# Mictronics/pluto-gps-sim

Hardware: AMD Instinct MI355X
Metric: IQ samples/sec (whole node) at 16 channels; bit-exact int16 IQ vs CPU ref (higher is better)
Workload: dtype f64 NCOs (exact), i32 accumulate of packed int16 I/Q

## Files before the change

### pluto-gps-sim_amd/csrc/gpsbb.hip

```cpp
#include <hip/hip_runtime.h>

#include <algorithm>
#include <atomic>
#include <cctype>
#include <cmath>
#include <cstdio>
#include <cstdlib>
#include <cstring>
#include <new>
#include <condition_variable>
#include <functional>
#include <mutex>
#include <thread>
#include <chrono>
#include <vector>

#include "gpsbb.h"
#include "gpsbb_kernels.hip.h"
#include "gpsbb_noise.hip.h"
#include "gpsbb_interf.hip.h"
#include "gpsbb_level.hip.h"
#include "gpsbb_events.hip.h"
#include "gpsbb_dense.hip.h"
#include "gpsbb_despread.hip.h"
#include "gpsbb_despread_lags.hip.h"
#include "gpsbb_acq.hip.h"
#include "gpsbb_track.hip.h"
#include "gpsbb_fir.hip.h"
#include "gpsbb_psd.hip.h"
#include "gpsbb_exc.hip.h"
#include "gpsbb_blank.hip.h"
#include "gpsbb_walk.hip.h"
#include "gpsbb_laps.hip.h"
#include "gpsbb_nco.h"
#include "gpsbb_testhooks.h"
#ifdef GPSBB_EXPERIMENTS
#include "gpsbb_modelerr.hip.h"
#endif

using namespace gpsbb_impl;

#ifdef GPSBB_EXPERIMENTS
#define GPSBB_KNOB_LONG(name, dflt) ([](long d) -> long { static const char *const e = getenv(name); return e ? atol(e) : d; }((long)(dflt)))
#define GPSBB_KNOB_SET(name) ([]() -> bool { static const bool v = getenv(name) != nullptr; return v; }())
#else
#define GPSBB_KNOB_LONG(name, dflt) ((long)(dflt))
#define GPSBB_KNOB_SET(name) (false)
#endif


namespace {

constexpr uint64_t kSinCosFnv1a = 0x1c99a5cf84551314ull;

bool make_sincos(int32_t sin512[512], int32_t cos512[512])
{
    const double two_pi = 6.283185307179586476925286766559;
    for (int i = 0; i < 512; i++) {
        const double a = two_pi * (double)i / 512.0;
        sin512[i] = (int32_t)(511.0 * std::sin(a) + 1.0);
        cos512[i] = (int32_t)(511.0 * std::cos(a) + 1.0);
    }
    uint64_t h = 0xcbf29ce484222325ull;
    auto eat = [&h](const int32_t *t) {
        for (int i = 0; i < 512; i++)
            for (int k = 0; k < 4; k++) {
                h ^= (uint8_t)((uint32_t)t[i] >> (8 * k));
                h *= 0x100000001b3ull;
            }
    };
    eat(sin512);
    eat(cos512);
    return h == kSinCosFnv1a;
}

const uint8_t kG2Taps[32][2] = {
    {2, 6}, {3, 7}, {4, 8}, {5, 9}, {1, 9}, {2, 10}, {1, 8}, {2, 9}, {3, 10}, {2, 3}, {3, 4},
    {5, 6}, {6, 7}, {7, 8}, {8, 9}, {9, 10}, {1, 4}, {2, 5}, {3, 6}, {4, 7}, {5, 8}, {6, 9},
    {1, 3}, {4, 6}, {5, 7}, {6, 8}, {7, 9}, {8, 10}, {1, 6}, {2, 7}, {3, 8}, {4, 9}};

void make_ca(int prn, uint8_t ca[GPSBB_CA_LEN])
{
    uint32_t g1 = 0x3ff, g2 = 0x3ff;
// ... 388 lines not shown
};

struct Event {
    hipEvent_t e = nullptr;
    hipError_t make(unsigned flags)
    {
        if (e)
            return hipSuccess;
        const hipError_t rc = hipEventCreateWithFlags(&e, flags);
        if (rc != hipSuccess)
            e = nullptr;
        else
            live_add(g_live_events, 1);
        return rc;
    }
    void release()
    {
        if (e) {
            (void)hipEventDestroy(e);
            live_add(g_live_events, -1);
        }
        e = nullptr;
    }
    operator hipEvent_t() const { return e; }
};

template <class... B>
static void release_all(B &...b)
{
    (b.release(), ...);
}

template <class F>
struct AtExit { F f; ~AtExit() { f(); } };
template <class F> AtExit(F) -> AtExit<F>;

struct KernelTimer {
    Event ev[2];
    hipError_t start(hipStream_t stream)
    {
#ifdef GPSBB_EXPERIMENTS
        for (Event &e : ev) {
            const hipError_t rc = e.make(hipEventDefault);
            if (rc != hipSuccess)
                return rc;
        }
        return hipEventRecord(ev[0], stream);
#else
        return hipSuccess;
#endif
    }
    hipError_t stop(hipStream_t stream)
    {
#ifdef GPSBB_EXPERIMENTS
        return hipEventRecord(ev[1], stream);
#else
        return hipSuccess;
#endif
    }
    float ms() const
    {
        float t = -1.0f;
        return ev[0] && ev[1] && hipEventElapsedTime(&t, ev[0], ev[1]) == hipSuccess ? t : -1.0f;
    }
    void release() { release_all(ev[0], ev[1]); }
};

struct gpsbb {
    int device = 0;
    hipStream_t s_seed = nullptr;
    hipStream_t s_more[SEED_STREAMS_MAX - 1] = {};
    unsigned batches_created = 0;
    hipStream_t s_compute = nullptr;
    hipStream_t s_compute2 = nullptr;
    unsigned compute_turn = 0;
    hipStream_t s_copy = nullptr;
    hipStream_t s_digest = nullptr;
    std::vector<uint32_t> h_ca;
    unsigned long long host_dwrd_oob = 0, host_itable_512 = 0;
    WorkPool *pool = nullptr;
    DevBuf<int32_t> d_tabs;
    DevBuf<uint32_t> d_ca;
    DevBuf<uint32_t> d_status;
    DevBuf<unsigned long long> d_hz;
    DevBuf<unsigned long long> d_clip;
    DevBuf<int2> d_noise_tab;
    DevBuf<unsigned long long> d_nclip;
    int last_hip = 0;
    gpsbb_batch *scratch = nullptr;
    PinnedBuf<unsigned char> h_bounce;
    PinnedBuf<unsigned char> h_fill;
    struct HostReg { char *host; char *dev; size_t bytes; };
    std::vector<HostReg> host_regs;
    struct ChainOnly *chain_only = nullptr;
    int sm_count = 0;
    int opt_seed_where = 0;
    int opt_synth_kernel = 0;
    int opt_skip_seed = 0;
    int opt_chain_where = 0;
    int last_kernel = 0;
    int last_variant = 0;
    int last_chain_dev = 0;
    int last_prepass = 0;
    DevBuf<unsigned char> d_pack;
    DevBuf<LevelOut> d_level;
    DevBuf<unsigned long long> d_digest;
    DevBuf<unsigned long long> d_acq_chips, d_acq_rows;
    DevBuf<unsigned long long> d_acq_grid;
    DevBuf<unsigned long long> d_trk;
    DevBuf<unsigned long long> d_fir;
    DevBuf<unsigned long long> d_psd_tab;
    DevBuf<unsigned long long> d_psd;
    DevBuf<unsigned long long> d_exc;
    DevBuf<unsigned long long> d_blank;
    KernelTimer acq_tm, trk_tm, fir_tm, psd_tm, exc_tm, blank_tm;
};

template <class F>
static void for_each_stream(const gpsbb *h, F f)
{
    for (hipStream_t st : {h->s_seed, h->s_compute, h->s_compute2, h->s_copy, h->s_digest})
        if (st)
            f(st);
    for (hipStream_t st : h->s_more)
        if (st)
            f(st);
}

static hipError_t drain_streams(const gpsbb *h)
{
    hipError_t first = hipSuccess;
    for_each_stream(h, [&](hipStream_t st) {
        const hipError_t e = hipStreamSynchronize(st);
        if (first == hipSuccess)
            first = e;
    });
    return first;
}

struct LapScratch {
    DevBuf<LapBC> bc;
    DevBuf<uint32_t> lane0, cnt, chunk_bad;
    DevBuf<LapRec> rec;
    DevBuf<LapAgg> agg;
    DevBuf<double> chunk_m;
    int reserve(size_t nbc, size_t nch, size_t nblocks, size_t chunks, bool room)
    {
        const size_t more = room ? chunks / 4 : 0;
        int e = bc.reserve(2 * nbc);
        e = e ? e : lane0.reserve(2 * nch * (nblocks + 1));
        e = e ? e : cnt.reserve(4 * GPSBB_MAX_CHAN);
        e = e ? e : rec.reserve(chunks * LAP_WG, room ? chunks * LAP_WG / 4 : 0);
        e = e ? e : agg.reserve(chunks, more);
        e = e ? e : chunk_m.reserve(chunks, more);
        return e ? e : chunk_bad.reserve(chunks, more);
    }
    void release() { release_all(bc, lane0, cnt, chunk_bad, rec, agg, chunk_m); }
    void dev(LapDev &L) const
    {
        L.bc = bc.p;
        L.lane0 = lane0.p;
        L.nlaps = cnt.p;
        L.nbad = cnt.p + 2 * GPSBB_MAX_CHAN;
        L.rec = rec.p;
        L.agg = agg.p;
        L.chunk_m = chunk_m.p;
// ... 242 lines not shown
        *out = (uint64_t)h->last_variant;
        return GPSBB_OK;
    case GPSBB_INFO_EXACT_RUNS:
    case GPSBB_INFO_CHAIN_FALLBACKS:
    case GPSBB_INFO_CHAIN_TIES:
    case GPSBB_INFO_CHAIN_REPAIRS:
    case GPSBB_INFO_TILES_RENDERED: {
        HIPCHK(h, hipSetDevice(h->device));
        unsigned long long v = 0;
        HIPCHK(h, hipMemcpy(&v, h->d_hz.p + (what == GPSBB_INFO_EXACT_RUNS ? 2 : (what == GPSBB_INFO_CHAIN_FALLBACKS ? 4 : (what == GPSBB_INFO_CHAIN_TIES ? 5 : (what == GPSBB_INFO_TILES_RENDERED ? 7 : 6)))), 8,
                            hipMemcpyDeviceToHost));
        *out = v;
        return GPSBB_OK;
    }
    case GPSBB_INFO_SC8_CLIPPED: {
        HIPCHK(h, hipSetDevice(h->device));
        unsigned long long v = 0;
        HIPCHK(h, hipMemcpy(&v, h->d_clip.p, 8, hipMemcpyDeviceToHost));
        *out = v;
        return GPSBB_OK;
    }
    case GPSBB_INFO_NOISE_CLIPPED: {
        unsigned long long v = 0;
        if (h->d_nclip.p) {
            HIPCHK(h, hipSetDevice(h->device));
            HIPCHK(h, hipMemcpy(&v, h->d_nclip.p, 8, hipMemcpyDeviceToHost));
        }
        *out = v;
        return GPSBB_OK;
    }
    case GPSBB_INFO_CHAIN_ON_DEVICE:
        *out = (uint64_t)h->last_chain_dev;
        return GPSBB_OK;
    case GPSBB_INFO_PREPASS:
        *out = (uint64_t)h->last_prepass;
        return GPSBB_OK;
    case GPSBB_INFO_STREAMS: {
        uint64_t n = 1;
        for_each_stream(h, [&](hipStream_t) { n++; });
        *out = n;
        return GPSBB_OK;
    }
    case GPSBB_INFO_HW_QUEUES: {
        const char *e = getenv("GPU_MAX_HW_QUEUES");
        const long v = e ? atol(e) : 4;
        *out = (uint64_t)(v > 0 ? v : 4);
        return GPSBB_OK;
    }
    default:
        return GPSBB_E_BADARG;
    }
}

extern "C" int gpsbb_codegen(int prn, uint8_t ca[GPSBB_CA_LEN])
{
    if (!ca || prn < 1 || prn > 32)
        return GPSBB_E_BADARG;
    make_ca(prn, ca);
    return GPSBB_OK;
}

extern "C" int gpsbb_sincos_tables(int32_t sin512[512], int32_t cos512[512])
{
    if (!sin512 || !cos512)
        return GPSBB_E_BADARG;
    return make_sincos(sin512, cos512) ? GPSBB_OK : GPSBB_E_INTERNAL;
}

static void chain_only_free(gpsbb *h);

extern "C" void gpsbb_destroy(gpsbb_t *h)
{
    if (!h)
        return;
    (void)hipSetDevice(h->device);
    if (h->scratch)
        gpsbb_batch_destroy(h->scratch);
    release_all(h->h_fill, h->h_bounce);
    for (const gpsbb::HostReg &r : h->host_regs)
        (void)hipHostUnregister(r.host);
    h->host_regs.clear();
    chain_only_free(h);
    (void)drain_streams(h);
    release_all(h->d_tabs, h->d_ca, h->d_status, h->d_hz, h->d_clip, h->d_noise_tab, h->d_nclip);
    release_all(h->d_pack, h->d_level, h->d_digest, h->d_acq_chips, h->d_acq_rows, h->d_acq_grid, h->d_trk, h->d_fir, h->d_psd_tab, h->d_psd, h->d_exc, h->d_blank);
    release_all(h->acq_tm, h->trk_tm, h->fir_tm, h->psd_tm, h->exc_tm, h->blank_tm);
    delete h->pool;
    h->pool = nullptr;
    for_each_stream(h, [](hipStream_t st) { (void)hipStreamDestroy(st); });
    delete h;
}

static hipError_t create_seed_stream(hipStream_t *st);

#ifdef GPSBB_EXPERIMENTS
__global__ void k_park(unsigned long long ticks)
{
    const unsigned long long t0 = wall_clock64();
    while (wall_clock64() - t0 < ticks)
        __builtin_amdgcn_s_sleep(64);
}
#endif

static hipError_t zero_now(gpsbb *h, void *ptr, size_t bytes)
{
#ifdef GPSBB_EXPERIMENTS
    {
        const long park = GPSBB_KNOB_LONG("GPSBB_X_PARK_NULL_MS", 0);
        if (park > 0)
            hipLaunchKernelGGL(k_park, dim3(1), dim3(1), 0, nullptr, (unsigned long long)park * 100000ull);
        if (GPSBB_KNOB_SET("GPSBB_X_NULL_MEMSET"))
            return hipMemsetAsync(ptr, 0, bytes, nullptr);
    }
#endif
    const hipError_t e = hipMemsetAsync(ptr, 0, bytes, h->s_seed);
    return e != hipSuccess ? e : hipStreamSynchronize(h->s_seed);
}

struct SynthKernel {
    void (*fn)(BatchDev, int16_t *);
    int lds;
};
static const SynthKernel &synth_kernel(int variant, bool digest, int g);

extern "C" int gpsbb_create(gpsbb_t **out, int device)
{
    if (!out)
        return GPSBB_E_BADARG;
    *out = nullptr;
    int ndev = 0;
    if (hipGetDeviceCount(&ndev) != hipSuccess || ndev <= 0 || device < 0 || device >= ndev)
        return GPSBB_E_NODEVICE;

    int32_t tabs[1024];
    if (!make_sincos(tabs + 512, tabs))
        return GPSBB_E_INTERNAL;
    std::vector<uint32_t> ca(33 * 32, 0u);
    for (int prn = 1; prn <= 32; prn++) {
        uint8_t chips[GPSBB_CA_LEN];
        make_ca(prn, chips);
        for (int i = 0; i < GPSBB_CA_LEN; i++)
            if (chips[i])
                ca[prn * 32 + (i >> 5)] |= 1u << (i & 31);
    }

    gpsbb *h = new (std::nothrow) gpsbb;
    if (!h)
        return GPSBB_E_NOMEM;
    h->device = device;
    auto fail = [&](hipError_t e) {
        h->last_hip = (int)e;
        gpsbb_destroy(h);
        return e == hipErrorOutOfMemory ? GPSBB_E_NOMEM : GPSBB_E_HIP;
    };
    hipError_t e;
    if ((e = hipSetDevice(device)) != hipSuccess) return fail(e);
    hipDeviceProp_t prop;
    if ((e = hipGetDeviceProperties(&prop, device)) != hipSuccess) return fail(e);
    h->sm_count = prop.multiProcessorCount;
    if ((e = create_seed_stream(&h->s_seed)) != hipSuccess) return fail(e);
    {
        const long sp = GPSBB_KNOB_LONG("GPSBB_SYNTH_STREAM_PRIO", 0);
        if (sp != 0) {
            if ((e = hipStreamCreateWithPriority(&h->s_compute, hipStreamNonBlocking, (int)sp)) != hipSuccess) return fail(e);
        } else {
            if ((e = hipStreamCreateWithFlags(&h->s_compute, hipStreamNonBlocking)) != hipSuccess) return fail(e);
        }
    }
    if ((e = create_seed_stream(&h->s_more[0])) != hipSuccess) return fail(e);
    if ((e = (hipError_t)h->d_tabs.reserve(sizeof tabs / sizeof tabs[0])) != hipSuccess) return fail(e);
    if ((e = (hipError_t)h->d_ca.reserve(ca.size())) != hipSuccess) return fail(e);
    if ((e = (hipError_t)h->d_status.reserve(1)) != hipSuccess) return fail(e);
    if ((e = (hipError_t)h->d_hz.reserve(8)) != hipSuccess) return fail(e);
    if ((e = (hipError_t)h->d_clip.reserve(1)) != hipSuccess) return fail(e);
    if ((e = hipMemcpy(h->d_tabs.p, tabs, sizeof tabs, hipMemcpyHostToDevice)) != hipSuccess) return fail(e);
    if ((e = hipMemcpy(h->d_ca.p, ca.data(), ca.size() * 4, hipMemcpyHostToDevice)) != hipSuccess) return fail(e);
    if ((e = hipStreamSynchronize(nullptr)) != hipSuccess) return fail(e);
    h->h_ca = ca;
    if ((e = zero_now(h, h->d_status.p, 4)) != hipSuccess) return fail(e);
    if ((e = zero_now(h, h->d_hz.p, h->d_hz.cap * sizeof *h->d_hz.p)) != hipSuccess) return fail(e);
    if ((e = zero_now(h, h->d_clip.p, 8)) != hipSuccess) return fail(e);
    for (int v = GPSBB_VARIANT_SYNTH; v <= GPSBB_VARIANT_EV_FIXED; v++)
        for (int dg = 0; dg < 2; dg++)
            for (int g = 0; g <= EV_STATE_LOG2_MAX; g++) {
                const SynthKernel &k = synth_kernel(v, dg != 0, g);
                if (k.fn && (e = hipFuncSetAttribute(reinterpret_cast<const void *>(k.fn), hipFuncAttributeMaxDynamicSharedMemorySize,
                                                     k.lds)) != hipSuccess) return fail(e);
            }
    *out = h;
    return GPSBB_OK;
}

typedef void (*LapKernelFn)(BatchDev, LapDev);
static LapKernelFn lap_pass2_kernel(int kind, bool wide, int g)
{
#define GPSBB_P2(W) {{k_lap_pass2<NCO_CODE, W, 0>, k_lap_pass2<NCO_CODE, W, 1>, k_lap_pass2<NCO_CODE, W, 2>}, \
                     {k_lap_pass2<NCO_CARR, W, 0>, k_lap_pass2<NCO_CARR, W, 1>, k_lap_pass2<NCO_CARR, W, 2>}, \
                     {k_lap_pass2_2<W, 0>, k_lap_pass2_2<W, 1>, k_lap_pass2_2<W, 2>}}
    static const LapKernelFn k[2][3][EV_STATE_LOG2_MAX + 1] = {GPSBB_P2(false), GPSBB_P2(true)};
#undef GPSBB_P2
    static_assert(NCO_CODE == 0 && NCO_CARR == 1, "lap_pass2_kernel's table");
    return k[wide ? 1 : 0][kind < 0 ? 2 : kind][g];
}

static const SynthKernel &synth_kernel(int variant, bool digest, int g)
{
#define GPSBB_SK(v, k) {k, synth_lds(v)}
#define GPSBB_SK1(v, k) {GPSBB_SK(v, k), {}, {}}
    static const SynthKernel k[GPSBB_VARIANT_EV_FIXED + 1][2][EV_STATE_LOG2_MAX + 1] = {
        {},
        {GPSBB_SK1(GPSBB_VARIANT_SYNTH, k_synth), {}},
        {{GPSBB_SK(GPSBB_VARIANT_EV, k_synth_ev<0>), GPSBB_SK(GPSBB_VARIANT_EV, k_synth_ev<1>), GPSBB_SK(GPSBB_VARIANT_EV, k_synth_ev<2>)},
         {GPSBB_SK(GPSBB_VARIANT_EV, k_synth_ev_digest<0>), GPSBB_SK(GPSBB_VARIANT_EV, k_synth_ev_digest<1>),
          GPSBB_SK(GPSBB_VARIANT_EV, k_synth_ev_digest<2>)}},
        {GPSBB_SK1(GPSBB_VARIANT_EV_DENSE, k_synth_ev_dense), {}},
        {GPSBB_SK1(GPSBB_VARIANT_PD_WIDE, k_synth_pd<true>), GPSBB_SK1(GPSBB_VARIANT_PD_WIDE, (k_synth_pd<true, true>))},
        {GPSBB_SK1(GPSBB_VARIANT_PD_NARROW, k_synth_pd<false>), GPSBB_SK1(GPSBB_VARIANT_PD_NARROW, (k_synth_pd<false, true>))},
        {GPSBB_SK1(GPSBB_VARIANT_EV_FIXED, k_synth_ev_fixed), {}},
    };
#undef GPSBB_SK1
#undef GPSBB_SK
    static_assert(GPSBB_VARIANT_SYNTH == 1 && GPSBB_VARIANT_EV == 2 && GPSBB_VARIANT_EV_DENSE == 3 && GPSBB_VARIANT_PD_WIDE == 4 &&
                      GPSBB_VARIANT_PD_NARROW == 5 && GPSBB_VARIANT_EV_FIXED == 6 && EV_STATE_LOG2_MAX == 2, "synth_kernel's table");
    return k[variant][digest ? 1 : 0][g];
}

static hipError_t stage_upload(gpsbb_batch *b, void *dst, const void *src, size_t bytes, hipStream_t stream)
{
    const size_t at = (b->stage_used + 63) & ~(size_t)63;
    if (at + bytes > b->stage.cap)
        return hipMemcpyAsync(dst, src, bytes, hipMemcpyHostToDevice, stream);
    memcpy(b->stage.p + at, src, bytes);
    b->stage_used = at + bytes;
    return hipMemcpyAsync(dst, b->stage.p + at, bytes, hipMemcpyHostToDevice, stream);
}


static int stage_arena(gpsbb_batch *b, size_t nbc)
{
    gpsbb *h = b->h;
    const size_t need = nbc * (sizeof(gpsbb_chan_t) + sizeof(EvConst) + 8 + 2 * 4 + 5 * 4 +
                               (size_t)CHAIN_SEG_MAX * (sizeof(ChainDesc) + 8 + 8 + 2 * 4)) + 64 * 1024;
    if (b->upload_done)
        HIPCHK(h, hipEventSynchronize(b->upload_done));
    PUSH_MARK("arena");
    HIPCHK(h, (hipError_t)b->stage.reserve(need, need / 4));
    b->stage_used = 0;
    return GPSBB_OK;
}

static int stage_plan(gpsbb_batch *b, hipStream_t upload_stream)
{
    gpsbb *h = b->h;
    const BatchPlan &pl = b->plan;
    const PlanImages &img = b->img;
// ... 363 lines not shown

}

static int host_seed_run(gpsbb_batch *b, const TableSet &ts, hipStream_t stream)
{
    const BatchPlan &pl = b->plan;
    gpsbb *h = b->h;
    const size_t nbc = (size_t)pl.nblocks * pl.nch;
    const size_t tr_n = 2 * nbc * ((size_t)pl.ntiles + 1);
    const size_t tx_n = 2 * nbc * (size_t)pl.ntiles, tn_n = nbc * (size_t)pl.ntiles;
    if (pl.ev) {
        HIPCHK(h, (hipError_t)b->hs_tile_x.reserve(tx_n, tx_n / 4));
        HIPCHK(h, (hipError_t)b->hs_tile_nav.reserve(tn_n, tn_n / 4));
    } else {
        HIPCHK(h, (hipError_t)b->hs_rows.reserve(pl.total_rows + 4, (pl.total_rows + 4) / 4));
        HIPCHK(h, (hipError_t)b->hs_tile_row.reserve(tr_n, tr_n / 4));
    }
    HIPCHK(h, (hipError_t)b->hs_end.reserve(nbc, nbc / 4));
    const size_t nchains = 2 * nbc;
    if (!h->pool) {
        const unsigned hw = std::thread::hardware_concurrency();
        size_t n = hw ? hw : 4;
        n = n > 32 ? 32 : n;
        h->pool = new (std::nothrow) WorkPool(n - 1);
        if (!h->pool)
            return GPSBB_E_NOMEM;
    }
    const size_t nthr = nchains;
    std::vector<unsigned long long> oob(nthr, 0ull), i512(nthr, 0ull);
    std::vector<char> ok(nthr, 1);
    h->pool->run(nchains, [&](size_t j) {
        const int kind = j < nbc ? 1 : 0;
        if (!host_seed_chain(b, kind, j < nbc ? j : j - nbc, &oob[j], &i512[j]))
            ok[j] = 0;
    });
    for (size_t t = 0; t < nthr; t++) {
        h->host_dwrd_oob += oob[t];
        h->host_itable_512 += i512[t];
        if (!ok[t])
            return GPSBB_E_INTERNAL;
    }
    if (pl.ev) {
        HIPCHK(h, hipMemcpyAsync(ts.tile_x.p, b->hs_tile_x.p, tx_n * sizeof(double), hipMemcpyHostToDevice, stream));
        HIPCHK(h, hipMemcpyAsync(ts.tile_nav.p, b->hs_tile_nav.p, tn_n * sizeof(uint32_t), hipMemcpyHostToDevice, stream));
    } else {
        HIPCHK(h, hipMemcpyAsync(ts.rows.p, b->hs_rows.p, pl.total_rows * sizeof(SynRow), hipMemcpyHostToDevice, stream));
        HIPCHK(h, hipMemcpyAsync(ts.tile_row.p, b->hs_tile_row.p, tr_n * sizeof(int32_t), hipMemcpyHostToDevice, stream));
    }
    HIPCHK(h, hipMemcpyAsync(ts.end.p, b->hs_end.p, nbc * sizeof(gpsbb_chan_state_t), hipMemcpyHostToDevice, stream));
    return GPSBB_OK;
}

static LaunchPlan batch_launch_plan(const gpsbb_batch *b, bool skip = false)
{
    return plan_launch(b->plan, LaunchIn{cu_count(b->h->sm_count), b->want_digest, b->link.d_carry != nullptr, skip}, launch_opts());
}

static BatchDev batch_dev(const gpsbb_batch *b, const TableSet &ts, const LaunchPlan &lp)
{
    const BatchPlan &pl = b->plan;
    const size_t set = (size_t)(&ts - b->sets);
    BatchDev p;
    memset(&p, 0, sizeof p);
    p.ch = b->d_ch.p;
    p.nblocks = pl.nblocks;
    p.nch = pl.nch;
    p.nsamp = pl.nsamp;
    p.ntiles = pl.ntiles;
    p.st_log2 = pl.st_log2;
    p.nstates = pl.nstates;
    p.delt = pl.delt;
    p.flags = pl.flags;
    p.tabs = b->h->d_tabs.p;
    p.ca_bits = b->h->d_ca.p;
    p.rows = reinterpret_cast<SynRow *>(ts.rows.p);
    p.row_off = b->d_row_off.p;
    p.tile_row = ts.tile_row.p;
    p.row_cnt = ts.row_cnt.p;
    p.tile_ctr = b->d_tile_ctr.p + set * ((size_t)pl.nblocks + 1);
    p.kph0 = (pl.flags & GPSBB_FIXED_CARRIER) ? b->d_kph0.p : nullptr;
    p.kstep = (pl.flags & GPSBB_FIXED_CARRIER) ? b->d_kstep.p : nullptr;
    p.end = ts.end.p;
    p.status = b->h->d_status.p;
    p.hazards = b->h->d_hz.p;
    p.digest = b->want_digest ? b->d_dig.p : nullptr;
    p.seed_order = b->d_seed_order.p;
    p.seed_lanes = lp.seed_lanes;
    p.ev = pl.ev ? 1 : 0;
    p.ev_chunk = lp.ev_chunk;
    p.pd_danger = lp.pd_danger;
    p.tile_x = ts.tile_x.p;
    p.tile_nav = ts.tile_nav.p;
    p.evc = b->d_evc.p;
    p.chain_dev = pl.chain_dev ? 1 : 0;
    p.chain_starts = pl.chain_starts ? 1 : 0;
    p.aux = pl.chain_dev ? ts.aux.p : nullptr;
    p.nseg = pl.nseg;
    p.seg_tiles = pl.seg_tiles;
    p.nvb = pl.nblocks * pl.nseg;
    p.fix_end = b->fix.end.p ? b->fix.end.p + set * GPSBB_MAX_CHAN * pl.fix_chunks : nullptr;
    p.fix_flag = b->fix.flag.p ? b->fix.flag.p + set * GPSBB_MAX_CHAN * pl.fix_chunks : nullptr;
    p.fix_epoch = b->fix.epoch;
    p.fix_chunks = pl.fix_chunks;
    p.model_start = pl.chain_model ? 1 : 0;
    p.cd = pl.chain_dev ? b->d_cd.p : nullptr;
    p.start0 = pl.chain_dev ? b->d_start0.p : nullptr;
    p.prefix_rows = pl.chain_dev && !pl.chain_starts ? ts.prefix.p : nullptr;
    p.carry = pl.chain_dev ? b->link.d_carry : nullptr;
    p.cont0_mask = pl.cont0_mask;
    p.lap_end = nullptr;
    return p;
}

static void lap_dev_plan(LapDev &L, const uint32_t chunk0[2][GPSBB_MAX_CHAN + 1], bool chained, size_t nbc)
{
    memcpy(L.chunk0, chunk0, sizeof L.chunk0);
    L.chained = chained ? 1 : 0;
    L.jitter = (uint32_t)GPSBB_KNOB_LONG("GPSBB_LAP_JITTER", 0);
    L.burst = GPSBB_KNOB_SET("GPSBB_LAP_NO_BURST") ? 0 : (int)GPSBB_KNOB_LONG("GPSBB_LAP_BURST_SHARE", LAP_BURST_SHARE);
    L.unit[NCO_CODE] = lap_unit(NCO_CODE, nbc);
    L.unit[NCO_CARR] = lap_unit(NCO_CARR, nbc);
}

static LapDev lap_dev(const gpsbb_batch *b, const TableSet &ts)
{
    const BatchPlan &pl = b->plan;
    LapDev L;
    ts.lap.dev(L);
    lap_dev_plan(L, pl.lap_chunk0, pl.chain_dev, (size_t)pl.nblocks * pl.nch);
    return L;
}

template <int KIND>
static void lap_chain_kind(hipStream_t ss, const BatchDev &p, const LapDev &L, int nch, LapKernelFn pass2)
{
    const unsigned chunks = L.chunk0[KIND][nch] - L.chunk0[KIND][0];
    hipLaunchKernelGGL(k_lap_plan<KIND>, dim3(nch), dim3(64), 0, ss, p, L);
    hipLaunchKernelGGL(k_lap_pass1<KIND>, dim3(chunks), dim3(LAP_WG), 0, ss, p, L);
    hipLaunchKernelGGL(k_lap_scan<KIND>, dim3(nch), dim3(64), 0, ss, p, L);
    hipLaunchKernelGGL(pass2, dim3(chunks), dim3(LAP_WG), 0, ss, p, L);
    hipLaunchKernelGGL(k_lap_repair<KIND>, dim3(nch), dim3(64), 0, ss, p, L);
}

static void lap_chain_launch(hipStream_t ss, const BatchDev &p, const LapDev &L, int nch, int kind, LapKernelFn pass2)
{
    if (kind == NCO_CODE) {
        lap_chain_kind<NCO_CODE>(ss, p, L, nch, pass2);
    } else if (kind == NCO_CARR) {
        lap_chain_kind<NCO_CARR>(ss, p, L, nch, pass2);
    } else {
        const unsigned chunks = L.chunk0[NCO_CODE][nch] - L.chunk0[NCO_CODE][0] + (L.chunk0[NCO_CARR][nch] - L.chunk0[NCO_CARR][0]);
        hipLaunchKernelGGL(k_lap_plan2, dim3(2 * nch), dim3(64), 0, ss, p, L);
        hipLaunchKernelGGL(k_lap_pass1_2, dim3(chunks), dim3(LAP_WG), 0, ss, p, L);
        hipLaunchKernelGGL(k_lap_scan2, dim3(2 * nch), dim3(64), 0, ss, p, L);
        hipLaunchKernelGGL(pass2, dim3(chunks), dim3(LAP_WG), 0, ss, p, L);
        hipLaunchKernelGGL(k_lap_repair2, dim3(2 * nch), dim3(64), 0, ss, p, L);
    }
}

static hipError_t walk_chain_launch(hipStream_t ss, const BatchDev &p, int carr_lanes, bool pass_a, int pass_b, int fix_wg,
                                    const CarryEvents &ce)
{
    hipError_t e;
    if (pass_a) {
        BatchDev pa = p;
        pa.seed_lanes = carr_lanes;
// ... 23 lines not shown
static int launch_events(gpsbb_batch *b, Event **ev)
{
    gpsbb *h = b->h;
    if (b->one_stream) {
        if (b->evs.empty())
            b->evs.emplace_back();
        b->ev_used = 0;
        *ev = b->evs[0].e;
        return GPSBB_OK;
    }
    if (b->ev_used == b->evs.size()) {
        if (b->evs.size() >= 4096) {
            b->ev_used = 0;
        } else {
            gpsbb_batch::Ev4 t;
            for (Event &e : t.e) {
                const hipError_t rc = e.make(hipEventDefault);
                if (rc != hipSuccess)
                    t.release();
                HIPCHK(h, rc);
            }
            b->evs.push_back(t);
        }
    }
    *ev = b->evs[b->ev_used++].e;
    return GPSBB_OK;
}

static int prepass_launch(gpsbb_batch *b, int set, const BatchDev &p, const LaunchPlan &lp, hipStream_t ss)
{
    const BatchPlan &pl = b->plan;
    gpsbb *h = b->h;
    const TableSet &ts = b->sets[set];
    const CarryEvents ce = {b->link.d_carry ? b->link.ev_prefix : nullptr, b->link.d_carry ? b->link.ev_fix : nullptr};
    if (lp.chain) {
        BatchDev pw = p;
        if (lp.chain_order) {
            pw.seed_order = b->d_chain_order.p;
            pw.seed_lanes = lp.walk_lanes;
        }
        HIPCHK(h, walk_chain_launch(ss, pw, lp.carr_lanes, lp.pass_a, lp.pass_b, lp.fix_wg, ce));
    }
    switch (lp.prepass) {
    case PREPASS_SKIP:
        break;
    case PREPASS_HOST: {
        const TableSet &prev = b->sets[(set + pl.nsets - 1) % pl.nsets];
        if (prev.synth_pending)
            HIPCHK(h, hipEventSynchronize(prev.synth_done_ref));
        return host_seed_run(b, ts, ss);
    }
    case PREPASS_LAPS: {
        const LapDev L = lap_dev(b, ts);
        if (!lp.lap_merged)
            lap_chain_launch(ss, p, L, pl.nch, NCO_CODE, lap_pass2_kernel(NCO_CODE, lp.lap_wide, lp.granule));
        if (lp.lap_fixed) {
            hipLaunchKernelGGL(k_lap_plan<NCO_CARR>, dim3(pl.nch), dim3(64), 0, ss, p, L);
            hipLaunchKernelGGL(k_lap_fixed_tiles, dim3(pl.nblocks * pl.nch), dim3(256), 0, ss, p);
        } else {
            const int kind = lp.lap_merged ? -1 : NCO_CARR;
            HIPCHK(h, ce.wait_both(ss));
            lap_chain_launch(ss, p, L, pl.nch, kind, lap_pass2_kernel(kind, lp.lap_wide, lp.granule));
            HIPCHK(h, ce.record_both(ss));
        }
        break;
    }
    case PREPASS_WALKS:
        if (!lp.chain)
            hipLaunchKernelGGL(k_walk<0>, dim3((lp.seed_lanes + GPSBB_WALK_WG - 1) / GPSBB_WALK_WG), dim3(GPSBB_WALK_WG), 0, ss, p);
        hipLaunchKernelGGL(k_tiles, dim3((1 + pl.nseg) * pl.nblocks * pl.nch), dim3(GPSBB_TILES_WG), 0, ss, p);
        break;
    case PREPASS_SEED: {
        const dim3 grid((lp.seed_lanes + GPSBB_SEED_WG - 1) / GPSBB_SEED_WG);
        if (lp.seed_ev)
            hipLaunchKernelGGL(k_seed<true>, grid, dim3(GPSBB_SEED_WG), 0, ss, p);
        else
            hipLaunchKernelGGL(k_seed<false>, grid, dim3(GPSBB_SEED_WG), 0, ss, p);
        break;
    }
    }
    return GPSBB_OK;
}

static int synth_launch(gpsbb_batch *b, const BatchDev &p, const LaunchPlan &lp, hipStream_t sc, int16_t *d_iq)
{
    const SynthKernel &k = synth_kernel(lp.variant, lp.digest_fused, lp.granule);
    hipLaunchKernelGGL(k.fn, dim3(lp.grid_x, lp.grid_y), dim3(lp.wg), k.lds, sc, p, d_iq);
    if (lp.digest_gx)
        hipLaunchKernelGGL(k_block_digest, dim3(lp.digest_gx, lp.digest_gy), dim3(256), 0, sc, (const uint32_t *)d_iq, b->plan.nsamp, b->d_dig.p);
    HIPCHK(b->h, hipGetLastError());
    return GPSBB_OK;
}

static int batch_launch(gpsbb_batch *b, int16_t *d_iq)
{
    const BatchPlan &pl = b->plan;
    gpsbb *h = b->h;
    const int set = (int)(b->run_count % (unsigned)pl.nsets);
    TableSet &ts = b->sets[set];
    b->fix.epoch++;
    if (b->want_digest)
        HIPCHK(h, (hipError_t)b->d_dig.reserve((size_t)pl.nblocks));
    const LaunchPlan lp = batch_launch_plan(b, h->opt_skip_seed && b->run_count >= (unsigned)pl.nsets);
    const BatchDev p = batch_dev(b, ts, lp);
    const bool timed = !b->one_stream;
    Event *ev = nullptr;
    int rc = launch_events(b, &ev);
    if (rc != GPSBB_OK)
        return rc;
    PUSH_MARK("l_ev");

    hipStream_t ss = nullptr;
    HIPCHK(h, batch_prepass_stream(b, pl.chain_dev, &ss));
    if (b->upload_done && b->upload_stream != ss)
        HIPCHK(h, hipStreamWaitEvent(ss, b->upload_done, 0));
    if (ts.synth_pending)
        HIPCHK(h, hipStreamWaitEvent(ss, ts.synth_done_ref, 0));
    if (timed)
        HIPCHK(h, hipEventRecord(ev[0], ss));
    rc = prepass_launch(b, set, p, lp, ss);
    if (rc != GPSBB_OK)
        return rc;
    HIPCHK(h, hipGetLastError());
    if (timed)
        HIPCHK(h, hipEventRecord(ev[1], ss));
    h->last_prepass = lp.info_prepass;
    h->last_kernel = lp.last_kernel;
    h->last_variant = lp.variant;
    h->last_chain_dev = lp.last_chain_dev;
    PUSH_MARK("l_pre");

    const bool one_cs = !GPSBB_KNOB_SET("GPSBB_TWO_COMPUTE_STREAMS");
    hipStream_t sc = h->s_compute;
    if (!one_cs && !b->one_stream && (pl.nsets >= 2 || b->max_sets == 1) && ((h->compute_turn++) & 1u)) {
        if (!h->s_compute2)
            HIPCHK(h, hipStreamCreateWithFlags(&h->s_compute2, hipStreamNonBlocking));
        sc = h->s_compute2;
    }
    b->last_cs = sc;
    if (sc != ss)
        HIPCHK(h, hipStreamWaitEvent(sc, ev[1], 0));
    if (!lp.ctr_reset)
        HIPCHK(h, hipMemsetAsync(p.tile_ctr, 0, ((size_t)pl.nblocks + 1) * sizeof(int32_t), sc));
    if (timed)
        HIPCHK(h, hipEventRecord(ev[2], sc));
    if (b->want_digest)
        HIPCHK(h, hipMemsetAsync(b->d_dig.p, 0, (size_t)pl.nblocks * sizeof(unsigned long long), sc));
    rc = synth_launch(b, p, lp, sc, d_iq);
    if (rc != GPSBB_OK)
        return rc;
    if (timed)
        HIPCHK(h, hipEventRecord(ev[3], sc));
    ts.synth_done_ref = ev[3];
    b->last_done = ev[3];
    ts.synth_pending = timed;
    b->last_set = set;
    b->run_count++;
    b->ran = true;
    return GPSBB_OK;
}

extern "C" int gpsbb_batch_run(gpsbb_batch_t *b, int16_t *d_iq)
{
    if (!b)
        return GPSBB_E_BADARG;
    gpsbb *h = b->h;
    HIPCHK(h, hipSetDevice(h->device));
    if (!d_iq) {
        HIPCHK(h, (hipError_t)b->d_iq.reserve((size_t)b->plan.nblocks * b->plan.nsamp * 2));
        d_iq = b->d_iq.p;
        b->last_iq = d_iq;
    } else {
        b->last_iq = nullptr;
        b->last_ext_iq = d_iq;
    }
    return batch_launch(b, d_iq);
}

extern "C" int16_t *gpsbb_batch_device_iq(gpsbb_batch_t *b) { return b ? b->last_iq : nullptr; }

extern "C" int gpsbb_sync(gpsbb_t *h)
{
    if (!h)
        return GPSBB_E_BADARG;
    HIPCHK(h, hipSetDevice(h->device));
    HIPCHK(h, drain_streams(h));
    uint32_t st = 0;
    HIPCHK(h, hipMemcpy(&st, h->d_status.p, 4, hipMemcpyDeviceToHost));
    if (st) {
        HIPCHK(h, zero_now(h, h->d_status.p, 4));
        return GPSBB_E_INTERNAL;
    }
    return GPSBB_OK;
}

extern "C" int gpsbb_batch_read(gpsbb_batch_t *b, int16_t *iq_out, gpsbb_chan_state_t *end_state)
{
    if (!b || !b->ran)
        return GPSBB_E_STATE;
    gpsbb *h = b->h;
    HIPCHK(h, hipSetDevice(h->device));
    if (iq_out) {
        const int16_t *src = b->last_iq ? b->last_iq : b->last_ext_iq;
        if (!src)
            return GPSBB_E_STATE;
        HIPCHK(h, hipMemcpy(iq_out, src, gpsbb_batch_iq_bytes(b), hipMemcpyDeviceToHost));
    }
    if (end_state)
        HIPCHK(h, hipMemcpy(end_state, b->sets[b->last_set].end.p, (size_t)b->plan.nblocks * b->plan.nch * sizeof(gpsbb_chan_state_t),
                            hipMemcpyDeviceToHost));
    return GPSBB_OK;
}

extern "C" int gpsbb_device_read(gpsbb_t *h, void *host_dst, const void *device_src, size_t bytes)
{
    if (!h || !host_dst || !device_src)
        return GPSBB_E_BADARG;
    HIPCHK(h, hipSetDevice(h->device));
    HIPCHK(h, hipMemcpy(host_dst, device_src, bytes, hipMemcpyDeviceToHost));
    return GPSBB_OK;
}

static int iq_call_begin(gpsbb *h, bool noise);

static int digest_blocks(gpsbb *h, hipStream_t stream, long wgs, const int16_t *d_iq, long nblocks, int nsamp, uint64_t *digest_out)
{
    HIPCHK(h, (hipError_t)h->d_digest.reserve((size_t)nblocks));
    HIPCHK(h, hipMemsetAsync(h->d_digest.p, 0, (size_t)nblocks * sizeof(unsigned long long), stream));
    long chunks = (wgs + nblocks - 1) / nblocks;
    const long max_chunks = ((long)nsamp + 1023) / 1024;
    chunks = chunks > max_chunks ? max_chunks : (chunks < 1 ? 1 : chunks);
    hipLaunchKernelGGL(k_block_digest, dim3((unsigned)chunks, (unsigned)nblocks), dim3(256), 0, stream, (const uint32_t *)d_iq, nsamp, h->d_digest.p);
    HIPCHK(h, hipGetLastError());
    HIPCHK(h, hipMemcpyAsync(digest_out, h->d_digest.p, (size_t)nblocks * sizeof(unsigned long long), hipMemcpyDeviceToHost, stream));
    HIPCHK(h, hipStreamSynchronize(stream));
    return GPSBB_OK;
}

extern "C" int gpsbb_device_digest(gpsbb_t *h, const int16_t *d_iq, long nblocks, int nsamp, uint64_t *digest_out)
{
    if (!h || !d_iq || !digest_out || nblocks < 1 || nblocks > 65535 || nsamp < 1)
        return GPSBB_E_BADARG;
    const int rc = iq_call_begin(h, false);
    return rc != GPSBB_OK ? rc : digest_blocks(h, h->s_compute, 2048, d_iq, nblocks, nsamp, digest_out);
}

extern "C" int gpsbb_slot_digest(gpsbb_t *h, const int16_t *d_iq, long nblocks, int nsamp, uint64_t *digest_out)
{
    if (!h || !d_iq || !digest_out || nblocks < 1 || nblocks > 65535 || nsamp < 1)
        return GPSBB_E_BADARG;
    HIPCHK(h, hipSetDevice(h->device));
    if (!h->s_digest)
        HIPCHK(h, hipStreamCreateWithFlags(&h->s_digest, hipStreamNonBlocking));
    return digest_blocks(h, h->s_digest, GPSBB_KNOB_LONG("GPSBB_SLOT_DIGEST_WGS", 2048), d_iq, nblocks, nsamp, digest_out);
}

extern "C" int gpsbb_get_hazards(gpsbb_t *h, gpsbb_hazards_t *out, int reset)
{
    if (!h || !out)
        return GPSBB_E_BADARG;
    HIPCHK(h, hipSetDevice(h->device));
    unsigned long long v[2];
    HIPCHK(h, hipMemcpy(v, h->d_hz.p, 16, hipMemcpyDeviceToHost));
    out->itable_512 = v[0];
    out->itable_512 += h->host_itable_512;
    out->dwrd_oob = v[1] + h->host_dwrd_oob;
    if (reset) {
        HIPCHK(h, zero_now(h, h->d_hz.p, 16));
        h->host_dwrd_oob = 0;
        h->host_itable_512 = 0;
    }
    return GPSBB_OK;
}
// ... 1278 lines not shown
    }
    HIPCHK(h, h->blank_tm.start(cs));
    hipLaunchKernelGGL(blank_kernel(ic.noise, ic.set), dim3((unsigned)nwg), dim3(BLANK_WG), blank_lds_bytes(K), cs, a);
    HIPCHK(h, hipGetLastError());
    hipLaunchKernelGGL(k_exc_fold, dim3(1), dim3(PSD_WG), 0, cs, a.part, h->d_blank.p + o_cnt, (int)nwg);
    HIPCHK(h, hipGetLastError());
    HIPCHK(h, h->blank_tm.stop(cs));
    uint32_t tail[GPSBB_BLANK_MAX_HIST];
    unsigned long long cnt[2] = {0, 0};
    HIPCHK(h, hipMemcpyAsync(cnt, h->d_blank.p + o_cnt, sizeof cnt, hipMemcpyDeviceToHost, cs));
    if (K > 0)
        HIPCHK(h, hipMemcpyAsync(tail, d_hout, (size_t)K * 4, hipMemcpyDeviceToHost, cs));
    HIPCHK(h, hipStreamSynchronize(cs));
    if (hist_out && K > 0)
        memcpy(hist_out, tail, (size_t)K * 4);
    if (blanked)
        *blanked = cnt[0];
    if (triggers)
        *triggers = cnt[1];
    return GPSBB_OK;
}

extern "C" double gpsbb_cn0_estimate(const gpsbb_corr_t *p, long n, long stride, double seg_seconds)
{
    if (!p || n < 2 || stride < 1 || !(seg_seconds > 0.0) || !std::isfinite(seg_seconds))
        return NAN;
    double mi = 0.0, mq = 0.0;
    for (long k = 0; k < n; k++) {
        mi += (double)p[k * stride].i;
        mq += (double)p[k * stride].q;
    }
    mi /= (double)n;
    mq /= (double)n;
    double vq = 0.0;
    for (long k = 0; k < n; k++) {
        const double d = (double)p[k * stride].q - mq;
        vq += d * d;
    }
    vq /= (double)(n - 1);
    if (!(mi > 0.0) || !(vq > 0.0))
        return NAN;
    return 10.0 * std::log10(mi * mi / (2.0 * seg_seconds * vq));
}

static int fill_block_finish(gpsbb_t *h, gpsbb_batch *b, int nch, int nsamp, int16_t *iq_out, gpsbb_chan_state_t *end_state,
                             const void *src, size_t bytes)
{
    const size_t end_bytes = (size_t)GPSBB_MAX_CHAN * sizeof(gpsbb_chan_state_t);
    HIPCHK(h, (hipError_t)h->h_fill.reserve(end_bytes + 64));
    hipStream_t cs = b->last_cs;
    uint32_t *st = reinterpret_cast<uint32_t *>(h->h_fill.p + end_bytes);
    *st = 0xffffffffu;
    if (GPSBB_KNOB_LONG("GPSBB_FILL_TAIL_KERNEL", 1) != 0) {
        static_assert(sizeof(gpsbb_chan_state_t) % 4 == 0, "copied as 32-bit words");
        hipLaunchKernelGGL(k_fill_tail, dim3(1), dim3(256), 0, cs, end_state ? b->sets[b->last_set].end.p : nullptr, h->d_status.p, h->h_fill.p, nch, st);
        HIPCHK(h, hipGetLastError());
    } else {
        if (end_state)
            HIPCHK(h, hipMemcpyAsync(h->h_fill.p, b->sets[b->last_set].end.p, (size_t)nch * sizeof(gpsbb_chan_state_t), hipMemcpyDeviceToHost, cs));
        HIPCHK(h, hipMemcpyAsync(st, h->d_status.p, 4, hipMemcpyDeviceToHost, cs));
    }
    PUSH_MARK("tail");
    bool bounce = false;
    if (iq_out) {
        const uintptr_t page = 4096, a = (uintptr_t)iq_out, e = a + bytes;
        for (const gpsbb::HostReg &r : h->host_regs) {
            const uintptr_t ra = (uintptr_t)r.host & ~(page - 1), re = ((uintptr_t)r.host + r.bytes + page - 1) & ~(page - 1);
            bounce = bounce || (a < re && ra < e);
        }
    }
    if (bounce) {
        HIPCHK(h, (hipError_t)h->h_bounce.reserve(bytes));
        HIPCHK(h, hipMemcpyAsync(h->h_bounce.p, src, bytes, hipMemcpyDeviceToHost, cs));
    } else if (iq_out) {
        HIPCHK(h, hipMemcpyAsync(iq_out, src, bytes, hipMemcpyDeviceToHost, cs));
    }
    PUSH_MARK("iq copy");
    HIPCHK(h, hipStreamSynchronize(cs));
    if (bounce)
        memcpy(iq_out, h->h_bounce.p, bytes);
    if (end_state)
        memcpy(end_state, h->h_fill.p, (size_t)nch * sizeof(gpsbb_chan_state_t));
    if (*st) {
        HIPCHK(h, zero_now(h, h->d_status.p, 4));
        return GPSBB_E_INTERNAL;
    }
    return GPSBB_OK;
}

extern "C" int gpsbb_host_register(gpsbb_t *h, void *ptr, size_t bytes)
{
    if (!h || !ptr || !bytes)
        return GPSBB_E_BADARG;
    HIPCHK(h, hipSetDevice(h->device));
    char *q = static_cast<char *>(ptr);
    for (const gpsbb::HostReg &r : h->host_regs)
        if (q < r.host + r.bytes && r.host < q + bytes)
            return GPSBB_E_STATE;
    HIPCHK(h, hipHostRegister(ptr, bytes, hipHostRegisterMapped));
    void *dev = nullptr;
    const hipError_t e = hipHostGetDevicePointer(&dev, ptr, 0);
    if (e != hipSuccess || !dev) {
        (void)hipHostUnregister(ptr);
        h->last_hip = (int)e;
        return GPSBB_E_HIP;
    }
    h->host_regs.push_back({q, static_cast<char *>(dev), bytes});
    return GPSBB_OK;
}

extern "C" int gpsbb_host_unregister(gpsbb_t *h, void *ptr)
{
    if (!h || !ptr)
        return GPSBB_E_BADARG;
    HIPCHK(h, hipSetDevice(h->device));
    for (size_t k = 0; k < h->host_regs.size(); k++)
        if (h->host_regs[k].host == static_cast<char *>(ptr)) {
            HIPCHK(h, drain_streams(h));
            HIPCHK(h, hipHostUnregister(ptr));
            h->host_regs.erase(h->host_regs.begin() + (long)k);
            return GPSBB_OK;
        }
    return GPSBB_E_STATE;
}

extern "C" int gpsbb_fill_block(gpsbb_t *h, const gpsbb_chan_t *ch, int nch, double delt, int nsamp,
                                int16_t *iq_out, gpsbb_chan_state_t *end_state)
{
    return gpsbb_fill_block_ex(h, ch, nch, delt, nsamp, 0u, iq_out, end_state);
}

static int fill_block_impl(gpsbb_t *h, const gpsbb_chan_t *ch, int nch, double delt, int nsamp, unsigned flags, const ImpairCall *ic,
                           int16_t *iq_out, gpsbb_chan_state_t *end_state)
{
    if (!h || !ch || !iq_out)
        return GPSBB_E_BADARG;
    HIPCHK(h, hipSetDevice(h->device));
    if (!h->scratch) {
        h->scratch = batch_new(h);
        if (!h->scratch)
            return GPSBB_E_NOMEM;
    }
    gpsbb_batch *b = h->scratch;
    int shift;
    const int fmt = out_format(flags, nsamp, &shift);
    if ((flags & 0xffu & ~GPSBB_FIXED_CARRIER & ~GPSBB_CHAIN_CARRIER) || fmt < 0)
        return GPSBB_E_BADARG;
    const size_t out_bytes = out_block_bytes(fmt, (size_t)nsamp);
    if (ic)
        HIPCHK(h, noise_ready(h));
    g_push_trace.start();
    b->one_stream = GPSBB_KNOB_LONG("GPSBB_FILL_ONE_STREAM", 1) != 0;
    int rc = batch_setup(b, PlanIn{ch, 1, nch, delt, nsamp, flags & GPSBB_FIXED_CARRIER}, plan_opts(h, b->max_sets), b->one_stream ? h->s_compute : h->s_seed);
    if (rc != GPSBB_OK)
        return rc;
    PUSH_MARK("set-up");
    int16_t *direct = nullptr;
    for (const gpsbb::HostReg &r : h->host_regs) {
        const char *q = reinterpret_cast<const char *>(iq_out);
        if (q >= r.host && (size_t)(q - r.host) <= r.bytes && out_bytes <= r.bytes - (size_t)(q - r.host)) {
            direct = reinterpret_cast<int16_t *>(r.dev + (q - r.host));
            break;
        }
    }
    rc = gpsbb_batch_run(b, (fmt || ic) ? nullptr : direct);
    if (rc != GPSBB_OK)
        return rc;
// ... 65 lines not shown
        for (int k = 0; k < GPSBB_N_DWRD; k++) {
            uint64_t w = 0;
            memcpy(&w, c + L->off_dwrd + (size_t)k * L->sizeof_dwrd_elem, L->sizeof_dwrd_elem);
            d[i].dwrd[k] = (uint32_t)w;
        }
        if (fixed && off_step != (size_t)-1 && std::isfinite(d[i].f_carr) && std::fabs(d[i].f_carr * delt) <= 0.125) {
            const volatile double scaled = 512.0 * 65536.0 * d[i].f_carr * delt;
            if (ld_i(c + off_step) != (int)std::round(scaled))
                return GPSBB_E_BADCHAN;
        }
    }
    int rc = gpsbb_fill_block_ex(h, d, max_chan, delt, nsamp, fixed ? GPSBB_FIXED_CARRIER : 0u, iq_buff, st);
    if (rc != GPSBB_OK)
        return rc;
    for (int i = 0; i < max_chan; i++) {
        if (d[i].prn <= 0)
            continue;
        char *c = base + (size_t)i * L->stride;
        if (fixed) {
            const unsigned ph = (unsigned)st[i].carr_phase;
            memcpy(c + L->off_carr_phase, &ph, 4);
        } else {
            memcpy(c + L->off_carr_phase, &st[i].carr_phase, 8);
        }
        memcpy(c + L->off_code_phase, &st[i].code_phase, 8);
        memcpy(c + L->off_iword, &st[i].iword, 4);
        memcpy(c + L->off_ibit, &st[i].ibit, 4);
        memcpy(c + L->off_icode, &st[i].icode, 4);
        memcpy(c + L->off_dataBit, &st[i].dataBit, 4);
        memcpy(c + L->off_codeCA, &st[i].codeCA, 4);
    }
    return GPSBB_OK;
}

extern "C" int gpsbb_fill_block_ref(gpsbb_t *h, void *chan, const gpsbb_refchan_layout_t *L, int max_chan,
                                    const double *gain, double delt, int nsamp, int16_t *iq_buff)
{
    return fill_block_ref(h, chan, L, false, (size_t)-1, max_chan, gain, delt, nsamp, iq_buff);
}

extern "C" int gpsbb_fill_block_ref_fixed(gpsbb_t *h, void *chan, const gpsbb_refchan_layout_t *L, size_t off_carr_phasestep,
                                          int max_chan, const double *gain, double delt, int nsamp, int16_t *iq_buff)
{
    return fill_block_ref(h, chan, L, true, off_carr_phasestep, max_chan, gain, delt, nsamp, iq_buff);
}


struct StreamChain {
    ChainCarry carry = {};
    int last_prn[GPSBB_MAX_CHAN] = {0};
    double rough_phase[GPSBB_MAX_CHAN] = {0};
    bool on_device = false;
    int fx_prn[GPSBB_MAX_CHAN] = {0};
    uint32_t fx_phase[GPSBB_MAX_CHAN] = {0};
    void forget(bool phases_too)
    {
        if (phases_too)
            *this = StreamChain();
        for (int i = 0; i < GPSBB_MAX_CHAN; i++)
            last_prn[i] = fx_prn[i] = carry.prn[i] = 0;
    }
};

struct gpsbb_stream {
    gpsbb *h = nullptr;
    int nch = 0, nsamp = 0, bps = 0, depth = 0;
    double delt = 0.0;
    unsigned flags = 0;
    int fmt = 0, shift = 0;
    bool noise_on = false;
    bool interf_on = false;
    ImpairArgs impair{};
    unsigned long long out_pos = 0;
    struct Slot {
        gpsbb_batch *batch = nullptr;
        PinnedBuf<unsigned char> h_iq;
        PinnedBuf<unsigned char> h_end;
        PinnedBuf<unsigned long long> h_dig;
        bool has_dig = false;
        DevBuf<LevelOut> d_lvl;
        PinnedBuf<LevelOut> h_lvl;
        bool has_lvl = false;
        Event computed, copied;
        void release()
        {
            if (batch)
                gpsbb_batch_destroy(batch);
            batch = nullptr;
            release_all(h_iq, h_dig, h_lvl, d_lvl, h_end, computed, copied);
        }
    };
    std::vector<Slot> slots;
    uint64_t head = 0, tail = 0;
    StreamChain chain;
    DevBuf<ChainCarryDev> d_carry;
    Event ev_prefix, ev_fix;
    std::vector<gpsbb_chan_t> seeded;
    std::vector<double> seeds;
    bool poisoned = false;
};

extern "C" void gpsbb_stream_destroy(gpsbb_stream_t *s)
{
    if (!s)
        return;
    (void)hipSetDevice(s->h->device);
    (void)drain_streams(s->h);
    release_all(s->d_carry, s->ev_prefix, s->ev_fix);
    for (auto &sl : s->slots)
        sl.release();
    delete s;
}

extern "C" int gpsbb_stream_create(gpsbb_t *h, int nch, double delt, int nsamp, int blocks_per_slot,
                                   int depth, unsigned flags, gpsbb_stream_t **out)
{
    if (!h || !out || nch < 1 || nch > GPSBB_MAX_CHAN || nsamp < 1 || blocks_per_slot < 1 || depth < 2 ||
        depth > 64 || !(delt > 0.0) || (flags & 0xffu & ~(GPSBB_CHAIN_CARRIER | GPSBB_FIXED_CARRIER | GPSBB_STREAM_DEVICE_ONLY)))
        return GPSBB_E_BADARG;
    int shift;
    const int fmt = out_format(flags, nsamp, &shift);
    if (fmt < 0 || (fmt && (flags & GPSBB_STREAM_DEVICE_ONLY)))
        return GPSBB_E_BADARG;
    *out = nullptr;
    HIPCHK(h, hipSetDevice(h->device));
    gpsbb_stream *s = new (std::nothrow) gpsbb_stream;
    if (!s)
        return GPSBB_E_NOMEM;
    s->h = h;
    s->nch = nch;
    s->nsamp = nsamp;
    s->bps = blocks_per_slot;
    s->depth = depth;
    s->delt = delt;
    s->flags = flags;
    s->fmt = fmt;
    s->shift = shift;
    s->slots.resize(depth);
    const size_t iq_bytes = (size_t)blocks_per_slot * nsamp * 4;
    const size_t host_bytes = (size_t)blocks_per_slot * out_block_bytes(fmt, (size_t)nsamp);
    const size_t end_bytes = (size_t)blocks_per_slot * nch * sizeof(gpsbb_chan_state_t);
    for (auto &sl : s->slots) {
        sl.batch = batch_new(h);
        hipError_t e = sl.batch ? hipSuccess : hipErrorOutOfMemory;
        if (e == hipSuccess && ((&sl - &s->slots[0]) & 1))
            e = use_second_seed_stream(sl.batch);
        if (e == hipSuccess) sl.batch->max_sets = 1;
        if (e == hipSuccess) e = (hipError_t)sl.batch->d_iq.reserve(iq_bytes / 2);
        if (e == hipSuccess && !(flags & GPSBB_STREAM_DEVICE_ONLY))
            e = (hipError_t)sl.h_iq.reserve(host_bytes);
        if (e == hipSuccess) e = (hipError_t)sl.h_end.reserve(end_bytes + 32);
        if (e == hipSuccess) e = sl.computed.make(hipEventDisableTiming);
        if (e == hipSuccess) e = sl.copied.make(hipEventDisableTiming);
        if (e != hipSuccess) {
            h->last_hip = (int)e;
            gpsbb_stream_destroy(s);
            return e == hipErrorOutOfMemory ? GPSBB_E_NOMEM : GPSBB_E_HIP;
        }
    }
    *out = s;
    return GPSBB_OK;
}

extern "C" int gpsbb_stream_pending(const gpsbb_stream_t *s) { return s ? (int)(s->head - s->tail) : 0; }

extern "C" int gpsbb_stream_reset(gpsbb_stream_t *s)
// ... 102 lines not shown
    if (s->interf_on) {
        c->a.it = s->impair.it;
        c->a.nz.shift = s->impair.it.shift;
    }
    return impair_at(c, s->out_pos, (uint64_t)s->bps * (uint64_t)s->nsamp);
}

static int push_level_memory(gpsbb_stream *s, const ImpairCall &ic)
{
    if (!level_fits(ic.a, ic.noise, s->nsamp))
        return GPSBB_E_BADARG;
    auto &sl = s->slots[s->head % s->depth];
    HIPCHK(s->h, hipSetDevice(s->h->device));
    HIPCHK(s->h, (hipError_t)sl.d_lvl.reserve((size_t)s->bps));
    HIPCHK(s->h, (hipError_t)sl.h_lvl.reserve((size_t)s->bps));
    return GPSBB_OK;
}

static int push_carry_to_device(gpsbb_stream *s, StreamChain &next)
{
    gpsbb *h = s->h;
    StreamChain &at = s->chain;
    if (!s->ev_fix) {
        hipError_t e = (hipError_t)s->d_carry.reserve(1);
        e = e ? e : zero_now(h, s->d_carry.p, sizeof(ChainCarryDev));
        e = e ? e : s->ev_prefix.make(hipEventDisableTiming);
        e = e ? e : s->ev_fix.make(hipEventDisableTiming);
        if (e != hipSuccess)
            release_all(s->d_carry, s->ev_prefix, s->ev_fix);
        HIPCHK(h, e);
    }
    if (!at.on_device && s->head > 0) {
        ChainCarryDev c;
        for (int i = 0; i < GPSBB_MAX_CHAN; i++)
            c.approx_end[i] = c.exact_end[i] = at.carry.phase[i];
        const int rc = gpsbb_sync(h);
        if (rc != GPSBB_OK)
            return rc;
        HIPCHK(h, hipMemcpy(s->d_carry.p, &c, sizeof c, hipMemcpyHostToDevice));
        HIPCHK(h, hipStreamSynchronize(nullptr));
        for (int i = 0; i < s->nch; i++) {
            at.last_prn[i] = at.carry.prn[i];
            at.rough_phase[i] = at.carry.phase[i];
        }
    }
    at.on_device = true;
    next = at;
    return GPSBB_OK;
}

static int push_carry_to_host(gpsbb_stream *s, StreamChain &next, PlanIn &in, PushSide &side)
{
    gpsbb *h = s->h;
    StreamChain &at = s->chain;
    if (at.on_device) {
        ChainCarryDev c;
        const int rc = gpsbb_sync(h);
        if (rc != GPSBB_OK)
            return rc;
        HIPCHK(h, hipMemcpy(&c, s->d_carry.p, sizeof c, hipMemcpyDeviceToHost));
        for (int i = 0; i < s->nch; i++) {
            at.carry.prn[i] = at.last_prn[i];
            at.carry.phase[i] = c.exact_end[i];
        }
        at.on_device = false;
    }
    next = at;
    const size_t nbc = (size_t)s->bps * s->nch;
    s->seeded.assign(in.ch, in.ch + nbc);
    s->seeds.resize(nbc);
    chain_carrier_host(in.ch, s->bps, s->nch, s->delt, s->nsamp, s->seeds.data(), 0, &next.carry);
    for (size_t k = 0; k < nbc; k++)
        s->seeded[k].carr_phase = s->seeds[k];
    in.ch = s->seeded.data();
    in.flags &= ~GPSBB_CHAIN_CARRIER;
    side.begun = false;
    return GPSBB_OK;
}

static int push_outputs(gpsbb_stream *s, gpsbb_stream::Slot &sl, ImpairCall &ic, bool want_digest, bool want_level)
{
    gpsbb *h = s->h;
    gpsbb_batch *b = sl.batch;
    hipStream_t cs = b->last_cs;
    if (sl.h_iq.p) {
        if (!h->s_copy)
            HIPCHK(h, hipStreamCreateWithFlags(&h->s_copy, hipStreamNonBlocking));
        cs = h->s_copy;
        HIPCHK(h, hipStreamWaitEvent(cs, b->last_done, 0));
    }
    PUSH_MARK("wait");
    if (sl.h_iq.p) {
        const bool sdma = GPSBB_KNOB_SET("GPSBB_GATHER_SDMA");
        if (sdma && !ic.any() && !s->fmt) {
            HIPCHK(h, hipMemcpyAsync(sl.h_iq.p, b->d_iq.p, (size_t)s->bps * s->nsamp * 4, hipMemcpyDeviceToHost, cs));
        } else {
            HIPCHK(h, out_launch(h, s->fmt, s->shift, ic.any() ? &ic : nullptr, b->d_iq.p, sl.h_iq.p, (size_t)s->bps * s->nsamp * 2, cs));
        }
    }
    PUSH_MARK("iq");
    const size_t bytes = (size_t)s->bps * s->nch * sizeof(gpsbb_chan_state_t);
    hipLaunchKernelGGL(k_end_states_to_host, dim3(64), dim3(256), 0, cs, (const uint4 *)b->sets[b->last_set].end.p,
                       (uint4 *)sl.h_end.p, (bytes + 15) / 16, h->d_status.p, (uint32_t *)(sl.h_end.p + ((bytes + 15) & ~(size_t)15)));
    HIPCHK(h, hipGetLastError());
    if (want_digest) {
        HIPCHK(h, hipMemcpyAsync(sl.h_dig.p, b->d_dig.p, (size_t)s->bps * sizeof(unsigned long long), hipMemcpyDeviceToHost, cs));
        sl.has_dig = true;
    }
    if (want_level) {
        HIPCHK(h, level_launch(h, ic.a, ic.noise, b->d_iq.p, s->bps, s->nsamp, sl.d_lvl.p, cs));
        HIPCHK(h, hipMemcpyAsync(sl.h_lvl.p, sl.d_lvl.p, (size_t)s->bps * sizeof(LevelOut), hipMemcpyDeviceToHost, cs));
        sl.has_lvl = true;
    }
    PUSH_MARK("endst");
    HIPCHK(h, hipEventRecord(sl.copied, cs));
    return GPSBB_OK;
}

struct PushGuard {
    gpsbb_stream *s;
    gpsbb_batch *b;
    bool queued = false, done = false;
    ~PushGuard()
    {
        b->link = StreamLink();
        s->poisoned = s->poisoned || (queued && !done);
    }
};

static int stream_push(gpsbb_stream_t *s, const gpsbb_chan_t *ch, bool new_chain, bool want_digest, bool want_level)
{
    if (!s || !ch)
        return GPSBB_E_BADARG;
    if (s->poisoned || s->head - s->tail >= (uint64_t)s->depth)
        return GPSBB_E_STATE;
    ImpairCall ic;
    if (!stream_impair(s, &ic))
        return GPSBB_E_BADARG;
    int rc = want_level ? push_level_memory(s, ic) : GPSBB_OK;
    if (rc != GPSBB_OK)
        return rc;
    if (new_chain)
        s->chain.forget(false);
    gpsbb *h = s->h;
    g_push_trace.start();
    HIPCHK(h, hipSetDevice(h->device));
    auto &sl = s->slots[s->head % s->depth];
    gpsbb_batch *b = sl.batch;
    const PlanOpts opts = plan_opts(h, b->max_sets);
    PlanIn in{ch, s->bps, s->nch, s->delt, s->nsamp, s->flags & (GPSBB_CHAIN_CARRIER | GPSBB_FIXED_CARRIER)};
    PushSide side;
    rc = plan_push_side(side, b->img, in, opts);
    if (rc != GPSBB_OK)
        return rc;
    StreamChain next = s->chain;
    if (side.chain == PUSH_CHAIN_DEVICE)
        rc = push_carry_to_device(s, next);
    else if (side.chain == PUSH_CHAIN_HOST)
        rc = push_carry_to_host(s, next, in, side);
    if (rc != GPSBB_OK)
        return rc;
    PushGuard guard{s, b};
    if (side.chain == PUSH_CHAIN_DEVICE) {
        b->link.d_carry = s->d_carry.p;
        b->link.carry_prn = s->chain.last_prn;
        b->link.carry_phase = next.rough_phase;
        b->link.ev_prefix = s->ev_prefix;
        b->link.ev_fix = s->ev_fix;
        b->link.stream_turn = (unsigned)s->head;
    }
    if ((s->flags & GPSBB_FIXED_CARRIER) && (s->flags & GPSBB_CHAIN_CARRIER) && s->head > 0) {
        b->link.fixed_prev_prn = s->chain.fx_prn;
        b->link.fixed_prev_phase = s->chain.fx_phase;
    }
    PUSH_MARK("plan");
    hipStream_t us = nullptr;
    HIPCHK(h, batch_prepass_stream(b, b->link.d_carry != nullptr, &us));
    rc = batch_setup(b, in, opts, us, side.begun ? &side.plan0 : nullptr);
    PUSH_MARK("setup");
    if (rc != GPSBB_OK)
        return rc;
    for (int i = 0; i < s->nch; i++) {
        const size_t k = (size_t)(s->bps - 1) * s->nch + i;
        if (side.chain == PUSH_CHAIN_DEVICE)
            next.last_prn[i] = in.ch[k].prn > 0 ? in.ch[k].prn : 0;
        if (s->flags & GPSBB_FIXED_CARRIER) {
            next.fx_prn[i] = in.ch[k].prn > 0 ? in.ch[k].prn : 0;
            next.fx_phase[i] = b->img.h_kph0[k] + (uint32_t)s->nsamp * (uint32_t)b->img.h_kstep[k];
        }
    }
    b->last_iq = b->d_iq.p;
    guard.queued = true;
    b->want_digest = want_digest;
    if (want_digest)
        HIPCHK(h, (hipError_t)sl.h_dig.reserve((size_t)s->bps));
    sl.has_dig = false;
    sl.has_lvl = false;
    rc = batch_launch(b, b->d_iq.p);
    PUSH_MARK("launch");
    if (rc != GPSBB_OK)
        return rc;
    PUSH_MARK("rec");
    rc = push_outputs(s, sl, ic, want_digest, want_level);
    if (rc != GPSBB_OK)
        return rc;
    s->chain = next;
    if (s->noise_on || s->interf_on)
        s->out_pos += (unsigned long long)s->bps * (unsigned long long)s->nsamp;
    s->head++;
    guard.done = true;
    g_push_trace.end();
    return GPSBB_OK;
}

extern "C" int gpsbb_stream_pop(gpsbb_stream_t *s, const int16_t **iq, gpsbb_chan_state_t *end_state)
{
    return gpsbb_stream_pop_digest(s, iq, end_state, nullptr);
}

static int stream_pop(gpsbb_stream_t *s, const int16_t **iq, gpsbb_chan_state_t *end_state, uint64_t *digests, gpsbb_level_t *levels);

extern "C" int gpsbb_stream_pop_digest(gpsbb_stream_t *s, const int16_t **iq, gpsbb_chan_state_t *end_state, uint64_t *digests)
{
    return stream_pop(s, iq, end_state, digests, nullptr);
}

extern "C" int gpsbb_stream_pop_level(gpsbb_stream_t *s, const int16_t **iq, gpsbb_chan_state_t *end_state, gpsbb_level_t *levels)
{
    return stream_pop(s, iq, end_state, nullptr, levels);
}

static int stream_pop(gpsbb_stream_t *s, const int16_t **iq, gpsbb_chan_state_t *end_state, uint64_t *digests, gpsbb_level_t *levels)
{
    if (!s || !iq)
        return GPSBB_E_BADARG;
    if (s->poisoned || s->head == s->tail)
        return GPSBB_E_STATE;
    if (digests && !s->slots[s->tail % s->depth].has_dig)
        return GPSBB_E_STATE;
    if (levels && !s->slots[s->tail % s->depth].has_lvl)
        return GPSBB_E_STATE;
    gpsbb *h = s->h;
    HIPCHK(h, hipSetDevice(h->device));
    auto &sl = s->slots[s->tail % s->depth];
    HIPCHK(h, hipEventSynchronize(sl.copied));
    *iq = sl.h_iq.p ? reinterpret_cast<const int16_t *>(sl.h_iq.p) : sl.batch->d_iq.p;
    if (end_state)
        memcpy(end_state, sl.h_end.p, (size_t)s->bps * s->nch * sizeof(gpsbb_chan_state_t));
    if (digests)
        memcpy(digests, sl.h_dig.p, (size_t)s->bps * sizeof(unsigned long long));
    if (levels)
        memcpy(levels, sl.h_lvl.p, (size_t)s->bps * sizeof(gpsbb_level_t));
    s->tail++;
    uint32_t st = 0;
    memcpy(&st, sl.h_end.p + (((size_t)s->bps * s->nch * sizeof(gpsbb_chan_state_t) + 15) & ~(size_t)15), 4);
    if (st) {
        HIPCHK(h, zero_now(h, h->d_status.p, 4));
        return GPSBB_E_INTERNAL;
    }
    return GPSBB_OK;
}


extern "C" int gpsbb_device_affinity(int device, int *numa_node, char *cpulist, size_t cpulist_cap)
{
    if (device < 0)
        return GPSBB_E_BADARG;
    int count = 0;
    if (hipGetDeviceCount(&count) != hipSuccess || device >= count)
        return GPSBB_E_NODEVICE;
    char bdf[64] = {0};
    if (hipDeviceGetPCIBusId(bdf, (int)sizeof bdf, device) != hipSuccess)
        return GPSBB_E_HIP;
    for (char *c = bdf; *c; c++)
        *c = (char)tolower((unsigned char)*c);
    if (numa_node)
        *numa_node = -1;
    if (cpulist && cpulist_cap)
        cpulist[0] = 0;
    char path[160];
    if (numa_node) {
        snprintf(path, sizeof path, "/sys/bus/pci/devices/%s/numa_node", bdf);
        if (FILE *f = fopen(path, "r")) {
            int v = -1;
            if (fscanf(f, "%d", &v) == 1)
                *numa_node = v;
            fclose(f);
        }
    }
    if (cpulist && cpulist_cap) {
        snprintf(path, sizeof path, "/sys/bus/pci/devices/%s/local_cpulist", bdf);
        if (FILE *f = fopen(path, "r")) {
            if (fgets(cpulist, (int)cpulist_cap, f)) {
                size_t n = strlen(cpulist);
                while (n && (cpulist[n - 1] == '\n' || cpulist[n - 1] == ' '))
                    cpulist[--n] = 0;
            } else {
                cpulist[0] = 0;
            }
            fclose(f);
        }
    }
    return GPSBB_OK;
}

static void chain_carrier_host(const gpsbb_chan_t *ch, int nblocks, int nch, double delt, int nsamp, double *seed,
                               int nthreads, ChainCarry *carry)
{
    auto work = [&](int i0, int i1) {
        for (int i = i0; i < i1; i++) {
            int prev_prn = carry ? carry->prn[i] : 0;
            double prev_x = carry ? carry->phase[i] : 0.0;
            for (int b = 0; b < nblocks; b++) {
                const gpsbb_chan_t &c = ch[(size_t)b * nch + i];
                double x0 = (c.prn > 0 && c.prn == prev_prn) ? prev_x : c.carr_phase;
                seed[(size_t)b * nch + i] = c.prn > 0 ? x0 : 0.0;
                if (c.prn > 0) {
                    volatile double s = c.f_carr * delt;
                    prev_x = carr_jump(x0, s, nsamp);
                }
                prev_prn = c.prn > 0 ? c.prn : 0;
            }
            if (carry) {
                carry->prn[i] = prev_prn;
                carry->phase[i] = prev_x;
            }
        }
    };
    if (nthreads <= 0 || nthreads > nch)
        nthreads = nch;
    if (nthreads == 1)
        work(0, nch);
    else
        channel_threads(nch, nthreads, work);
}

extern "C" int gpsbb_chain_carrier_host(const gpsbb_chan_t *ch, int nblocks, int nch, double delt, int nsamp,
                                        double *seed, int nthreads)
{
    if (!ch || !seed || nblocks < 1 || nch < 1 || nch > GPSBB_MAX_CHAN || nsamp < 1 || !(delt > 0.0))
// ... 471 lines not shown
    HIPCHK(h, hipMemcpy(he.data(), p.end, ne * sizeof(gpsbb_chan_state_t), hipMemcpyDeviceToHost));
    out[0] = out[1] = out[2] = 0;
    std::vector<gpsbb_chan_t> hc(ne);
    HIPCHK(h, hipMemcpy(hc.data(), p.ch, ne * sizeof(gpsbb_chan_t), hipMemcpyDeviceToHost));
    for (size_t k = 0; k < ne; k++) {
        if (hc[k].prn <= 0)
            continue;
        const size_t blk = k / (size_t)pl.nch, i = k % (size_t)pl.nch;
        if (ev_nav_in_sign(pl.st_log2)) {
            unsigned long long *x = &hx[ev_tile_x_row(blk, pl.nch, (int)i, NCO_CODE, nst)];
            uint32_t *nv = &hn[ev_tile_nav_row(blk, pl.nch, (int)i, nst)];
            const uint32_t nav_end = nav_pack(he[k].icode, he[k].ibit, he[k].iword);
            uint32_t after = nav_bit(hc[k].dwrd, nav_advance(nav_end)) < 0 ? 1u : 0u;
            uint32_t next_bit = he[k].dataBit < 0 ? 1u : 0u;
            unsigned long long next_mag;
            memcpy(&next_mag, &he[k].code_phase, 8);
            for (int e = nst - 1; e >= 0; e--) {
                const uint32_t here = ev_state_bit(x[e]);
                x[e] = ev_state_mag(x[e]);
                if (next_mag < x[e])
                    after = next_bit;
                nv[e] = here | (after << 1);
                next_bit = here;
                next_mag = x[e];
            }
        }
        for (int kind = 0; kind < 2; kind++)
            for (int t = 0; t < pl.ntiles; t += 1 << ev_kind_log2(kg, kind)) {
                const size_t at = ev_tile_x_row(blk, pl.nch, (int)i, kind, pl.ntiles) + t;
                out[0] += mix(hx[ev_tile_x_row(blk, pl.nch, (int)i, kind, nst) + ev_state_at(pl.st_log2, kind, t).entry] +
                              0x9E3779B97F4A7C15ull * (at + 1));
            }
        for (int t = 0; t < pl.ntiles; t += 1 << kg) {
            const size_t at = ev_tile_nav_row(blk, pl.nch, (int)i, pl.ntiles) + t;
            out[1] += mix((unsigned long long)(hn[ev_tile_nav_row(blk, pl.nch, (int)i, nst) + ev_state_at(pl.st_log2, NCO_CODE, t).entry] & 3u) +
                          0x9E3779B97F4A7C15ull * (at + 1));
        }
        unsigned long long w[5];
        memcpy(w, &he[k], sizeof w);
        for (int q = 0; q < 4; q++)
            out[2] += mix(w[q] + 0x9E3779B97F4A7C15ull * (k * 5 + q + 1));
        out[2] += mix((unsigned long long)(uint32_t)he[k].codeCA + 0x9E3779B97F4A7C15ull * (k * 5 + 5));
    }
    return GPSBB_OK;
}

extern "C" void gpsbb_test_budgets(double out[3])
{
    out[0] = EV_MODEL_ERR * 0x1p+32;
    out[1] = EV_T_EPS * 0x1p+32;
    out[2] = (double)PD_BAND;
}

extern "C" unsigned long long gpsbb_test_row_bound(int kind, double s_abs, int nsamp)
{
    return kind == NCO_CODE ? row_bound(s_abs, 1023.0, 9, nsamp) : row_bound(s_abs, 1.0, -1, nsamp);
}

extern "C" long long gpsbb_test_read_pattern(gpsbb_t *h, const void *d_src, size_t bytes)
{
    if (!h || !d_src)
        return GPSBB_E_BADARG;
    const int rows = 32, cols = 2442;
    const size_t per_wave = (size_t)rows * cols * 8;
    size_t waves = bytes / per_wave;
    waves -= waves % 4;
    if (waves < 4)
        return GPSBB_E_BADARG;
    DevBuf<double> d_sink;
    if (d_sink.reserve(1) != hipSuccess)
        return GPSBB_E_NOMEM;
    hipLaunchKernelGGL(k_read_pattern, dim3((unsigned)(waves / 4)), dim3(256), 0, h->s_compute, (const double *)d_src, rows, cols, d_sink.p);
    const hipError_t e = hipStreamSynchronize(h->s_compute);
    d_sink.release();
    return e == hipSuccess ? (long long)(waves * per_wave) : (long long)GPSBB_E_HIP;
}

extern "C" unsigned long long gpsbb_test_despread_exact(gpsbb_batch *b) { return b ? b->ds_last_exact : 0ull; }
extern "C" float gpsbb_test_despread_ms(gpsbb_batch *b) { return b ? b->ds_tm.ms() : -1.0f; }
extern "C" float gpsbb_test_acquire_ms(gpsbb *h) { return h ? h->acq_tm.ms() : -1.0f; }
extern "C" float gpsbb_test_track_ms(gpsbb *h) { return h ? h->trk_tm.ms() : -1.0f; }
extern "C" float gpsbb_test_fir_ms(gpsbb *h) { return h ? h->fir_tm.ms() : -1.0f; }

extern "C" int gpsbb_test_fir_tile(void) { return FIR_TILE; }
extern "C" float gpsbb_test_psd_ms(gpsbb *h) { return h ? h->psd_tm.ms() : -1.0f; }
extern "C" int gpsbb_test_psd_run(int log2n) { return log2n < PSD_MIN_LOG2N || log2n > PSD_MAX_LOG2N ? -1 : psd_min_run(log2n); }
extern "C" float gpsbb_test_exc_ms(gpsbb *h) { return h ? h->exc_tm.ms() : -1.0f; }
extern "C" int gpsbb_test_exc_run(int log2n) { return log2n < EXC_MIN_LOG2N || log2n > EXC_MAX_LOG2N ? -1 : exc_min_run(log2n); }
extern "C" int gpsbb_test_exc_host(const gpsbb_exc_t *e, const int16_t *w, long nsamp, const int16_t *hist_in, int16_t *out, int16_t *hist_out,
                                   uint64_t *clipped, uint64_t *excised, int64_t *peak)
{
    if (!e || e->log2n < EXC_MIN_LOG2N || e->log2n > EXC_MAX_LOG2N)
        return GPSBB_E_BADARG;
    std::vector<psd_c> work((size_t)1 << e->log2n), half((size_t)1 << (e->log2n - 1), psd_c{0, 0});
    return exc_host(e, w, nsamp, hist_in, psd_table(), psd_table() + PSD_TW, work.data(), half.data(), out, hist_out, clipped, excised, peak)
               ? GPSBB_OK
               : GPSBB_E_BADARG;
}
extern "C" float gpsbb_test_blank_ms(gpsbb *h) { return h ? h->blank_tm.ms() : -1.0f; }
extern "C" void gpsbb_test_blank_nt(int on) { g_blank_nt = on != 0; }
extern "C" int gpsbb_test_blank_tile(int *run)
{
    if (run)
        *run = BLANK_MIN_RUN;
    return BLANK_TILE;
}
extern "C" int gpsbb_test_blank_host(const gpsbb_blank_t *b, const int16_t *w, long nsamp, const int16_t *hist_in, int16_t *out, int16_t *hist_out,
                                     uint64_t *blanked, uint64_t *triggers)
{
    return blank_host(b, w, nsamp, hist_in, out, hist_out, blanked, triggers) ? GPSBB_OK : GPSBB_E_BADARG;
}

#ifdef GPSBB_WG_TRACE
namespace {
DevBuf<unsigned long long> g_trace_buf;
unsigned g_trace_cap = 0;
}
extern "C" int gpsbb_test_wg_trace_begin(unsigned cap)
{
    if (hipDeviceSynchronize() != hipSuccess)
        return GPSBB_E_HIP;
    if (cap > g_trace_cap) {
        g_trace_cap = 0;
        g_trace_buf.release();
        if (g_trace_buf.reserve((size_t)cap * WG_TRACE_WORDS) != hipSuccess)
            return GPSBB_E_NOMEM;
        g_trace_cap = cap;
    }
    const unsigned zero = 0;
    if (hipMemcpyToSymbol(HIP_SYMBOL(g_wg_trace), &g_trace_buf.p, sizeof g_trace_buf.p) != hipSuccess ||
        hipMemcpyToSymbol(HIP_SYMBOL(g_wg_trace_cap), &cap, sizeof cap) != hipSuccess ||
        hipMemcpyToSymbol(HIP_SYMBOL(g_wg_trace_n), &zero, sizeof zero) != hipSuccess)
        return GPSBB_E_HIP;
    return hipDeviceSynchronize() == hipSuccess ? GPSBB_OK : GPSBB_E_HIP;
}
extern "C" long gpsbb_test_wg_trace_read(unsigned long long *out, unsigned cap)
{
    if (hipDeviceSynchronize() != hipSuccess)
        return GPSBB_E_HIP;
    unsigned n = 0;
    if (hipMemcpyFromSymbol(&n, HIP_SYMBOL(g_wg_trace_n), sizeof n) != hipSuccess)
        return GPSBB_E_HIP;
    const unsigned have = n < g_trace_cap ? n : g_trace_cap, take = have < cap ? have : cap;
    if (take && hipMemcpy(out, g_trace_buf.p, (size_t)take * WG_TRACE_WORDS * 8, hipMemcpyDeviceToHost) != hipSuccess)
        return GPSBB_E_HIP;
    return (long)n;
}
#endif
#endif
```

### pluto-gps-sim_amd/csrc/gpsbb_events.hip.h

```cpp
#ifndef GPSBB_EVENTS_HIP_H
#define GPSBB_EVENTS_HIP_H

#include <cstddef>
#include <type_traits>

#include "gpsbb_kernels.hip.h"

namespace gpsbb_impl {

#ifndef GPSBB_EV_WG
#define GPSBB_EV_WG 1024
#endif
constexpr int EV_WG = GPSBB_EV_WG;
constexpr int EV_WAVES = EV_WG / 64;
constexpr int EV_KC_MAX = 4;
constexpr int EV_AMP_PAD = EV_KC_MAX;
constexpr int EV_AMP_STRIDE = 512 + EV_AMP_PAD + 4;
constexpr int EV_CHIP_LEN = 1024 + 544;
constexpr int EV_KC_DENSE = EV_KC_MAX + 1;
#ifndef GPSBB_EV_CHUNK
#define GPSBB_EV_CHUNK 4
#endif
constexpr int EV_CHUNK = GPSBB_EV_CHUNK;
constexpr int PD_CHUNK = 2;
// ... 463 lines not shown
        GPSBB_EV_OUT(i1, h1, mb)
        asm("v_add3_u32 %0, %1, %2, %3" : "=v"(msum) : "v"(msum), "v"(ma), "v"(mb));
    }
    if (mask) {
        const int i0 = __builtin_ctz(mask);
        GPSBB_EV_IN(i0)
        EvHalf<KC> h0 = ev_first<KC, FIXED>(L, i0, Ki0, xti0, yti0, tki0, tci0, off);
        uint32_t ma;
        GPSBB_EV_OUT(i0, h0, ma)
        msum += ma;
    }
#undef GPSBB_EV_IN
#undef GPSBB_EV_OUT
#undef GPSBB_EV_STATES
}

constexpr int EV_PICK_LDS = 16;
static_assert(sizeof(EvLds) + EV_PICK_LDS <= 160 * 1024 && sizeof(EvLdsLean) + EV_PICK_LDS <= 160 * 1024, "one workgroup per CU: 160 KB of LDS");
constexpr int EV_HELP_SCAN = 64 * 64;
__device__ __forceinline__ int ev_pick_block(const BatchDev &p, uint32_t slot)
{
    const int wg = (int)blockIdx.x;
    if (wg < p.nblocks)
        return wg;
    int b = -1;
    if (threadIdx.x < 64) {
        const int lane = (int)threadIdx.x;
        int ticket = 0;
        if (lane == 0)
            ticket = __hip_atomic_fetch_add(p.tile_ctr + p.nblocks, 1, __ATOMIC_RELAXED, __HIP_MEMORY_SCOPE_AGENT);
        ticket = __builtin_amdgcn_readfirstlane(ticket);
        const int live_upto = p.ntiles - EV_WAVES * p.ev_chunk;
        const int nscan = p.nblocks < EV_HELP_SCAN ? p.nblocks : EV_HELP_SCAN;
        unsigned long long mymask = 0ull;
        int nlive = 0;
        for (int c = 0; c * 64 < nscan; c++) {
            const int pos = c * 64 + lane;
            const bool live = pos < nscan &&
                              __hip_atomic_load(p.tile_ctr + (p.nblocks - 1 - (pos < nscan ? pos : 0)), __ATOMIC_RELAXED, __HIP_MEMORY_SCOPE_AGENT) <= live_upto;
            const unsigned long long m = __builtin_amdgcn_ballot_w64(live);
            if (lane == c)
                mymask = m;
            nlive += __popcll(m);
        }
        if (nlive > 0) {
            const int r = ticket % nlive;
            const int cnt = __popcll(mymask);
            int incl = cnt;
#pragma unroll
            for (int d = 1; d < 64; d <<= 1) {
                const int v = __shfl_up(incl, d);
                if (lane >= d)
                    incl += v;
            }
            const unsigned long long hm = __builtin_amdgcn_ballot_w64(r >= incl - cnt && r < incl);
            const int c = __builtin_amdgcn_readfirstlane((int)__ffsll((long long)hm) - 1);
            const uint32_t lo = (uint32_t)__shfl((int)(uint32_t)mymask, c), hi = (uint32_t)__shfl((int)(uint32_t)(mymask >> 32), c);
            unsigned long long cm = ((unsigned long long)hi << 32) | lo;
            int k = __builtin_amdgcn_readfirstlane(r - __shfl(incl - cnt, c));
            for (; k > 0; k--)
                cm &= cm - 1ull;
            b = p.nblocks - 1 - (c * 64 + (int)__ffsll((long long)cm) - 1);
        }
        if (lane == 0)
            lds_write_at<int>(slot, b);
    }
    __syncthreads();
    return __builtin_amdgcn_readfirstlane(lds_read_at<int>(slot));
}

template <bool DENSE, bool FIXED = false, bool DIGEST = false, int SG = 0>
__device__ __forceinline__ void synth_ev_body(const BatchDev &p, int16_t *__restrict__ iq)
{
    extern __shared__ __attribute__((aligned(16))) unsigned char smem_raw[];
    typedef typename std::conditional<DENSE, EvLds, EvLdsLean>::type LDS;
    LDS &L = *reinterpret_cast<LDS *>(smem_raw);

    const int tid = threadIdx.x;
#ifdef GPSBB_EV_PRIO
    __builtin_amdgcn_s_setprio(GPSBB_EV_PRIO);
#endif
    if (lds_addr_of(smem_raw) != 0u) {
        if (tid == 0)
            atomicOr(p.status, ST_LDS_LAYOUT);
        return;
    }
#ifdef GPSBB_WG_TRACE
    WgTrace wgt = wg_trace_enter();
#endif
    const int b = ev_pick_block(p, (uint32_t)sizeof(LDS));
#ifdef GPSBB_WG_TRACE
    wgt.block = b;
    wgt.nblocks = p.nblocks;
#endif
    if (b < 0) {
#ifdef GPSBB_WG_TRACE
        wg_trace_leave(wgt, wgt.wall0, wgt.clk0, 0u, 1u, false);
#endif
        return;
    }
    const gpsbb_chan_t *__restrict__ cb = p.ch + (size_t)b * p.nch;
    const EvConst *__restrict__ kb = p.evc + (size_t)b * p.nch;
    for (int i = __builtin_amdgcn_readfirstlane(tid >> 6); i < p.nch; i += EV_WAVES) {
        const int prn = cb[i].prn;
        const bool down = kb[i].down != 0;
        const double g = cb[i].gain;
        int32_t tc[(LDS::AMP + 63) / 64], ts[(LDS::AMP + 63) / 64];
#pragma unroll
        for (int j = 0; j < (LDS::AMP + 63) / 64; j++) {
            const int e = (tid & 63) + 64 * j;
            const int k = down ? 511 - (e & 511) : (e & 511);
            tc[j] = p.tabs[k];
            ts[j] = p.tabs[512 + k];
        }
        const uint32_t my_word = p.ca_bits[(prn > 0 ? prn : 0) * 32 + (tid & 31)];
#pragma unroll
        for (int j = 0; j < (LDS::AMP + 63) / 64; j++) {
            const int e = (tid & 63) + 64 * j;
            uint32_t v = 0;
            if (prn > 0) {
                const int ip = (int)mul_rn((double)tc[j], g);
                const int qp = (int)mul_rn((double)ts[j], g);
                v = ((uint32_t)qp << 16) + (uint32_t)ip;
            }
            if (e < LDS::AMP)
                L.amp[i][e] = v;
        }
#pragma unroll 4
        for (int j = 0; j < (LDS::CHIPS + 63) / 64; j++) {
            const int c = (tid & 63) + 64 * j;
            const int ca = c >= GPSBB_CA_LEN ? c - GPSBB_CA_LEN : c;
            const int cb1 = c + 1 >= GPSBB_CA_LEN ? c + 1 - GPSBB_CA_LEN : c + 1;
            const uint32_t w0 = (uint32_t)__shfl((int)my_word, (ca >> 5) & 31), w1 = (uint32_t)__shfl((int)my_word, (cb1 >> 5) & 31);
            uint32_t v = 0;
            if (prn > 0) {
                const uint32_t b0 = (w0 >> (ca & 31)) & 1u;
                const uint32_t b1 = (w1 >> (cb1 & 31)) & 1u;
                v = (b0 ? 0x00u : 0xffu) | (b0 == b1 ? 0x0f00u : 0x0000u);
            }
            if (c < LDS::CHIPS)
                L.chip2[i][c] = (uint16_t)v;
        }
    }
    for (int e = tid; e < EV_WAVES * 16 * 64; e += EV_WG)
        (&L.D[0][0][0])[e] = 0u;
    {
        const int l = tid & 63;
        if (l < p.nch) {
            L.tstate[tid >> 6][1][2 * l] = kb[l].tC0;
            L.tstate[tid >> 6][1][2 * l + 1] = kb[l].tK0;
        }
        if (SG && tid < 2 * p.nch)
            L.tstep[tid] = (tid & 1) ? kb[tid >> 1].S : kb[tid >> 1].sc;
    }
    __syncthreads();
#ifdef GPSBB_WG_TRACE
    const unsigned long long t_staged = wall_clock64(), c_staged = clock64();
#endif

    const int wave = __builtin_amdgcn_readfirstlane(tid >> 6), lane = tid & 63;
    const int ntw = p.ntiles;
    const int nch2 = 2 * p.nch;
    uint32_t mk[EV_KC_MAX];
    uint32_t mkd;
    {
        const bool act = lane < p.nch && cb[lane < p.nch ? lane : 0].prn > 0;
        const int kc = act ? kb[lane].kc : 0;
// ... 264 lines not shown
```

### pluto-gps-sim_amd/csrc/gpsbb_kernels.hip.h

```cpp
#ifndef GPSBB_KERNELS_HIP_H
#define GPSBB_KERNELS_HIP_H

#include <hip/hip_runtime.h>
#include <stdint.h>

#include "gpsbb.h"
#include "gpsbb_nco.h"

namespace gpsbb_impl {

#ifndef GPSBB_WG
#define GPSBB_WG 512
#endif
#ifndef GPSBB_WAVES_PER_SIMD
#define GPSBB_WAVES_PER_SIMD 4
#endif
constexpr int TILE_THREADS = GPSBB_WG;
#ifndef GPSBB_SPT
#define GPSBB_SPT 16
#endif
constexpr int SPT = GPSBB_SPT;
constexpr int TILE = 64 * SPT;
constexpr int WAVES_PER_WG = TILE_THREADS / 64;
#ifndef GPSBB_TILE_CHUNK
#define GPSBB_TILE_CHUNK 2
#endif
constexpr int TILE_CHUNK = GPSBB_TILE_CHUNK;
#ifndef GPSBB_ROW_CAP
#define GPSBB_ROW_CAP 128
#endif
constexpr int WAVE_ROW_CAP = GPSBB_ROW_CAP;

constexpr uint32_t ST_ROW_OVERFLOW = 1u;
constexpr uint32_t ST_LDS_LAYOUT = 4u;
constexpr uint32_t ST_CHAIN_STALL = 2u;

struct SynRow {
    int32_t n0;
    uint32_t nav;
    double x;
    double S;
};
static_assert(sizeof(SynRow) == sizeof(NcoRow), "row pool is sized for NcoRow");

struct EvConst {
    double S;
    double rS;
    double sc;
    double rsc;
    uint32_t danger_le;
    uint32_t chip_at;
    uint32_t amp_at;
    uint32_t danger;
    double tK0;
    double tC0;
    double W;
    int32_t kc;
    int32_t down;
    double pd_S8;
    double pd_dy;
    double pd_sc2;
    double pd_dx;
    uint32_t _pad[4];
};
static_assert(sizeof(EvConst) == 128 && offsetof(EvConst, danger_le) == 32, "EvConst layout");

constexpr int CHAIN_MAX_CROSS = 20;
constexpr int CHAIN_PREFIX_CAP = 64;
struct ChainAux {
    double start1;
    double endA;
    double margin;
    int32_t ncross;
    int32_t cross[CHAIN_MAX_CROSS];
    uint32_t hz512;
    int32_t wrap_row;
    int32_t prefix_cnt, prefix_end;
    int32_t _pad;
    double pre[CHAIN_MAX_CROSS], post[CHAIN_MAX_CROSS];
    double endB;
    double seg[CHAIN_MAX_CROSS + 1];
    double wrap_x;
};

struct ChainDesc {
    double f_carr;
    double carr_phase;
    int32_t prn;
    int32_t start;
};
static_assert(sizeof(ChainDesc) == 24, "ChainDesc layout");

struct ChainCarryDev {
    double approx_end[GPSBB_MAX_CHAN];
    double exact_end[GPSBB_MAX_CHAN];
};

#ifdef GPSBB_WG_TRACE
constexpr int WG_TRACE_WORDS = 12;
__device__ unsigned long long *g_wg_trace;
__device__ unsigned g_wg_trace_cap, g_wg_trace_n;
struct WgTrace {
    unsigned long long wall0, clk0;
    int block;
    int nblocks;
};
__device__ __forceinline__ WgTrace wg_trace_enter()
{
    WgTrace t;
    t.wall0 = wall_clock64();
    t.clk0 = clock64();
    t.block = (int)blockIdx.x;
    t.nblocks = 0;
    return t;
}
__device__ __forceinline__ void wg_trace_leave(const WgTrace &t, unsigned long long wall_staged, unsigned long long clk_staged, unsigned tiles,
                                               unsigned kind, bool worked)
{
    const unsigned long long wall_loop = wall_clock64(), clk_loop = clock64();
    if (worked)
        __syncthreads();
    if (threadIdx.x == 0 && g_wg_trace) {
        const unsigned k = atomicAdd(&g_wg_trace_n, 1u);
        if (k < g_wg_trace_cap) {
            unsigned long long *r = g_wg_trace + (size_t)k * WG_TRACE_WORDS;
            r[0] = t.wall0;
            r[1] = wall_staged;
            r[2] = wall_loop;
            r[3] = wall_clock64();
            r[4] = t.clk0;
            r[5] = clk_staged;
            r[6] = clk_loop;
            r[7] = clock64();
            r[8] = (unsigned long long)__builtin_amdgcn_s_getreg(4 | (31 << 11))  |
                   ((unsigned long long)__builtin_amdgcn_s_getreg(20 | (31 << 11))  << 32);
            r[9] = (unsigned long long)(uint32_t)(t.block & 0xffffff) | ((unsigned long long)(t.nblocks && (int)blockIdx.x >= t.nblocks ? 1u : 0u) << 24) |
                   ((unsigned long long)tiles << 40);
            r[10] = kind | (worked ? 0x100u : 0u);
            r[11] = (unsigned long long)(uint32_t)t.nblocks | ((unsigned long long)gridDim.x << 32);
        }
    }
}
#endif

struct BatchDev {
    const gpsbb_chan_t *ch;
    int nblocks, nch, nsamp, ntiles;
    double delt;
    unsigned flags;
    const int32_t *tabs;
    const uint32_t *ca_bits;
    SynRow *rows;
    const uint64_t *row_off;
    int32_t *tile_row;
    int32_t *row_cnt;
    gpsbb_chan_state_t *end;
    int32_t *tile_ctr;
    const uint32_t *kph0;
    const int32_t *kstep;
    int seed_lanes;
    const int32_t *seed_order;
    uint32_t *status;
    unsigned long long *digest;
    unsigned long long *hazards;
    int ev;
    int ev_chunk;
    int st_log2;
    int nstates;
    uint32_t pd_danger;
    double *tile_x;
    uint32_t *tile_nav;
    const EvConst *evc;
    int chain_dev;
    int chain_starts;
    ChainAux *aux;
    int nseg, seg_tiles, nvb;
    int model_start;
    ChainDesc *cd;
    const double *start0;
    SynRow *prefix_rows;
    ChainCarryDev *carry;
    unsigned long long *fix_end;
    int *fix_flag;
    int fix_epoch, fix_chunks;
    uint32_t cont0_mask;
    double *lap_end;
};

__device__ __forceinline__ int seg_nsamp(const BatchDev &p, int sgi)
{
    const int n0 = sgi * p.seg_tiles * TILE;
    const int left = p.nsamp - n0;
    const int full = p.seg_tiles * TILE;
    return p.nseg <= 1 ? p.nsamp : (left < full ? left : full);
}

__device__ __forceinline__ size_t tile_row_at(const BatchDev &p, int b, int t, int i, int kind)
{
    return ((size_t)b * (p.ntiles + 1) + t) * (2 * p.nch) + 2 * i + kind;
}
__device__ __forceinline__ int chain_code(const BatchDev &p, int b, int i) { return b * p.nch + i; }
__device__ __forceinline__ int chain_carr(const BatchDev &p, int b, int i) { return p.nblocks * p.nch + b * p.nch + i; }

template <class P>
__host__ __device__ __forceinline__ int nav_bit(const P dwrd, uint32_t nav)
{
    int w = nav_iword(nav);
    w = w < GPSBB_N_DWRD ? w : GPSBB_N_DWRD - 1;
    return (int)((dwrd[w] >> (29 - nav_ibit(nav))) & 1u) * 2 - 1;
}

__device__ __forceinline__ uint64_t readlane_u64(uint64_t v, int src)
{
    const uint32_t lo = (uint32_t)__builtin_amdgcn_readlane((int)(uint32_t)v, src);
    const uint32_t hi = (uint32_t)__builtin_amdgcn_readlane((int)(uint32_t)(v >> 32), src);
    return ((uint64_t)hi << 32) | lo;
}


struct RowSink {
    SynRow *rows;
    uint32_t cap;
    uint32_t cnt;
    bool overflow;
    unsigned long long *hz;
    const uint32_t *dwrd;
    uint32_t dbit;
    int32_t *tile_row;
    uint32_t tr;
    uint32_t tstride;
    int32_t tile_t;
    int32_t ntiles;
    int32_t wrap_pend;

    __device__ __forceinline__ void row(int32_t n0, uint32_t nav, double x, double S, bool after_wrap)
    {
        {
            const int32_t nt = (int32_t)(((uint32_t)n0 + (uint32_t)(TILE - 1)) / (uint32_t)TILE);
            const int32_t lim = nt < ntiles ? nt : ntiles;
            const int32_t here = (int32_t)(cnt < cap ? cnt : cap);
            while (tile_t < lim) {
                tile_row[tr] = (here - 1) | wrap_pend;
                wrap_pend = 0;
                tr += tstride;
                tile_t++;
// ... 111 lines not shown
            atomicAdd(hz + 1, 1ull);
#else
            hz_local[1]++;
#endif
        }
        dbit = nav_bit(dwrd, nav) < 0 ? 0x80000000u : 0u;
    }
    GPSBB_HD void finish() { flush(INT32_MAX - TILE); }
};

GPSBB_HD TileSink make_tile_sink(double *tile_x, uint32_t *tile_nav, int nch, int ntiles, int b, int i, int kind,
                                 const uint32_t *dwrd, uint32_t nav0, unsigned long long *hz)
{
    TileSink s;
    s.tx = tile_x + ((size_t)b * (2 * (size_t)nch) + 2 * i + kind) * (size_t)ntiles;
    s.tn = kind == 0 ? tile_nav + ((size_t)b * (size_t)nch + i) * (size_t)ntiles : nullptr;
    s.tile_t = 0;
    s.ntiles = ntiles;
    s.pn0 = 0;
    s.px = s.pS = 0.0;
    s.pbits = 0;
    s.cnt = 0;
    s.overflow = false;
    s.hz = hz;
    s.hz_local[0] = s.hz_local[1] = 0;
    s.dwrd = dwrd;
    s.dbit = dwrd && nav_bit(dwrd, nav0) < 0 ? 0x80000000u : 0u;
    return s;
}

struct ChainDone {
    const SynRow *rows;
    int cnt;
};

__device__ __forceinline__ RowSink make_sink(const BatchDev &p, int chain, const uint32_t *dwrd, uint32_t nav0)
{
    RowSink s;
    const uint64_t o0 = p.row_off[chain], o1 = p.row_off[chain + 1];
    s.rows = p.rows + o0;
    s.cap = (uint32_t)(o1 - o0 - 1);
    s.cnt = 0;
    s.overflow = false;
    s.hz = p.hazards;
    s.dwrd = dwrd;
    s.dbit = dwrd && nav_bit(dwrd, nav0) < 0 ? 0x80000000u : 0u;
    const int nbc = p.nblocks * p.nch;
    const int kind = chain >= nbc ? 1 : 0, bi = chain - kind * nbc;
    s.tile_row = p.tile_row;
    s.tr = (uint32_t)tile_row_at(p, bi / p.nch, 0, bi % p.nch, kind);
    s.tstride = 2u * (uint32_t)p.nch;
    s.tile_t = 0;
    s.ntiles = p.ntiles;
    s.wrap_pend = 0;
    return s;
}

template <bool EV>
__device__ inline ChainDone seed_code_chain(const BatchDev &p, int b, int i)
{
    const gpsbb_chan_t &c = p.ch[(size_t)b * p.nch + i];
    gpsbb_chan_state_t &e = p.end[(size_t)b * p.nch + i];
    ChainDone d = {nullptr, 0};
    if (c.prn <= 0) {
        e.code_phase = 0.0;
        e.iword = e.ibit = e.icode = e.dataBit = e.codeCA = 0;
        e._pad = 0;
        return d;
    }
    const int chain = chain_code(p, b, i);
    uint32_t nav = nav_pack(c.icode, c.ibit, c.iword);
    const double s = mul_rn(c.f_code, p.delt);
    double x;
    if (EV) {
        TileSink sink = make_tile_sink(p.tile_x, p.tile_nav, p.nch, p.ntiles, b, i, 0, c.dwrd, nav, p.hazards);
        x = build_rows_f64<NCO_CODE>(c.code_phase, s, nav, p.nsamp, sink);
        sink.finish();
        d.cnt = (int)sink.cnt;
    } else {
        RowSink sink = make_sink(p, chain, c.dwrd, nav);
        x = build_rows_f64<NCO_CODE>(c.code_phase, s, nav, p.nsamp, sink);
        sink.finish();
        if (sink.overflow)
            atomicOr(p.status, ST_ROW_OVERFLOW);
        d.rows = sink.rows;
        d.cnt = (int)sink.cnt;
    }
    e.code_phase = x;
    e.iword = nav_iword(nav);
    e.ibit = nav_ibit(nav);
    e.icode = nav_icode(nav);
    e.dataBit = nav_bit(c.dwrd, nav);
    const int ci = (int)x;
    e.codeCA = (int)((p.ca_bits[c.prn * 32 + (ci >> 5)] >> (ci & 31)) & 1u) * 2 - 1;
    e._pad = 0;
    return d;
}

template <bool EV>
__device__ inline ChainDone seed_carr_chain(const BatchDev &p, int b, int i, double x0, double *x_end)
{
    const gpsbb_chan_t &c = p.ch[(size_t)b * p.nch + i];
    gpsbb_chan_state_t &e = p.end[(size_t)b * p.nch + i];
    ChainDone d = {nullptr, 0};
    if (c.prn <= 0) {
        e.carr_phase = 0.0;
        *x_end = 0.0;
        return d;
    }
    const int chain = chain_carr(p, b, i);
    uint32_t nav = 0;
    const double s = mul_rn(c.f_carr, p.delt);
    double x;
    if (EV) {
        TileSink sink = make_tile_sink(p.tile_x, p.tile_nav, p.nch, p.ntiles, b, i, 1, nullptr, 0u, p.hazards);
        x = build_rows_f64<NCO_CARR>(x0, s, nav, p.nsamp, sink);
        sink.finish();
        d.cnt = (int)sink.cnt;
    } else {
        RowSink sink = make_sink(p, chain, nullptr, 0u);
        x = build_rows_f64<NCO_CARR>(x0, s, nav, p.nsamp, sink);
        sink.finish();
        if (sink.overflow)
            atomicOr(p.status, ST_ROW_OVERFLOW);
        d.rows = sink.rows;
        d.cnt = (int)sink.cnt;
    }
    e.carr_phase = x;
    *x_end = x;
    return d;
}

GPSBB_HD double fixed_tile_index(uint32_t ph0, int32_t step, int t)
{
    const uint32_t ph = ph0 + (uint32_t)t * (uint32_t)TILE * (uint32_t)step;
    return (double)(ph & 0x1ffffffu) * 0x1p-16;
}

__device__ inline void seed_carr_fixed(const BatchDev &p, int b, int i)
{
    const size_t k = (size_t)b * p.nch + i;
    p.row_cnt[chain_carr(p, b, i)] = 0;
    p.end[k].carr_phase = p.ch[k].prn > 0 ? (double)(uint32_t)(p.kph0[k] + (uint32_t)p.nsamp * (uint32_t)p.kstep[k]) : 0.0;
}

#ifndef GPSBB_SEED_WG
#define GPSBB_SEED_WG 256
#endif
#ifndef GPSBB_SEED_PRIO
#define GPSBB_SEED_PRIO 3
#endif
template <bool EV>
__global__ __launch_bounds__(GPSBB_SEED_WG) void k_seed(BatchDev p)
{
    __builtin_amdgcn_s_setprio(GPSBB_SEED_PRIO);
    const int gid = blockIdx.x * blockDim.x + threadIdx.x;
    if (gid >= p.seed_lanes)
        return;
    const int c = p.seed_order[gid];
    if (c < 0)
        return;
    const int nbc = p.nblocks * p.nch;
    if (c < nbc) {
        const ChainDone d = seed_code_chain<EV>(p, c / p.nch, c % p.nch);
        if (!EV)
            p.row_cnt[chain_code(p, c / p.nch, c % p.nch)] = d.cnt;
        return;
    }
    const int g = c - nbc, b = g / p.nch, i = g % p.nch;
    if (p.kph0) {
        seed_carr_fixed(p, b, i);
        return;
    }
    double unused;
    const ChainDone d = seed_carr_chain<EV>(p, b, i, p.ch[(size_t)b * p.nch + i].carr_phase, &unused);
    if (!EV)
        p.row_cnt[chain_carr(p, b, i)] = d.cnt;
}


typedef short v2s __attribute__((ext_vector_type(2)));

__device__ __forceinline__ v2s u32_v2s(uint32_t u)
{
    v2s v;
    __builtin_memcpy(&v, &u, 4);
    return v;
}
__device__ __forceinline__ uint32_t v2s_u32(v2s v)
{
    uint32_t u;
    __builtin_memcpy(&u, &v, 4);
    return u;
}

struct __attribute__((aligned(16))) WaveRows {
    uint4 a[WAVE_ROW_CAP];
    uint32_t s_lo[WAVE_ROW_CAP];
    uint32_t s_hi[WAVE_ROW_CAP];
};

struct SynthLds {
    uint32_t amp[GPSBB_MAX_CHAN][512];
    int8_t chip[GPSBB_MAX_CHAN][1024];
    uint32_t dwrd[GPSBB_MAX_CHAN][GPSBB_N_DWRD];
    double sc[GPSBB_MAX_CHAN];
    double rsc[GPSBB_MAX_CHAN];
// ... 452 lines not shown
                1, CARR, if (!last) {                                                                                  \
                    half_ok = nc + nk <= 64;                                                                           \
                    if (half_ok)                                                                                       \
                        prefetch_channel(W, lane, readlane_u64(tile_addr, 2 * a + 2), readlane_u64(tile_addr, 2 * a + 3), \
                                         nc, nk, 64 * ((a + 1) & 1));                                                  \
                } else if (more) GPSBB_STAGE_NEXT_TILE)                                                                \
        }                                                                                                              \
        remaining = 0;                                                                                                 \
    }

            if (ovf) {
                if (fixed_carr)
                    GPSBB_DENSE_TILE(2)
                else
                    GPSBB_DENSE_TILE(1)
            } else if (fixed_carr) {
                GPSBB_CHANNEL(2, 2, m_c2)
                GPSBB_CHANNEL(0, 2, m_c0)
                GPSBB_CHANNEL(1, 2, m_c1)
            } else {
                GPSBB_CHANNEL(2, 0, m_c2 & ~m_k1)
                GPSBB_CHANNEL(0, 0, m_c0 & ~m_k1)
                GPSBB_CHANNEL(2, 1, m_c2 & m_k1)
                GPSBB_CHANNEL(0, 1, m_c0 & m_k1)
                GPSBB_CHANNEL(1, 0, m_c1 & ~m_k1)
                GPSBB_CHANNEL(1, 1, m_c1 & m_k1)
            }
            if (more && nact == 0)
                GPSBB_STAGE_NEXT_TILE
#undef GPSBB_CHANNEL
#undef GPSBB_DENSE_TILE
#undef GPSBB_LOOKUP_AND_WALK
#undef GPSBB_STAGE_NEXT_TILE
            if (more) {
                asm volatile("s_waitcnt vmcnt(0)" ::: "memory");
                slot_n0a = (int)W.a[lane].x;
                slot_n0b = (int)W.a[64 + lane].x;
                cur = nxt;
                cwrap = nwrap;
            }

            uint32_t *out = reinterpret_cast<uint32_t *>(iq) + (size_t)b * p.nsamp + n0;
            if (nvalid == SPT && ((reinterpret_cast<uintptr_t>(out) & 15u) == 0)) {
                uint4 *o4 = reinterpret_cast<uint4 *>(out);
#pragma unroll
                for (int j = 0; j < SPT; j += 4)
                    o4[j >> 2] = make_uint4(v2s_u32(acc[j]), v2s_u32(acc[j + 1]), v2s_u32(acc[j + 2]), v2s_u32(acc[j + 3]));
            } else {
#pragma unroll
                for (int j = 0; j < SPT; j++)
                    if (j < nvalid)
                        out[j] = v2s_u32(acc[j]);
            }
        }
    }
}

__global__ __launch_bounds__(256) void k_read_pattern(const double *__restrict__ src, int rows, int cols, double *__restrict__ sink)
{
    const int wave = (int)((blockIdx.x * blockDim.x + threadIdx.x) >> 6), lane = (int)(threadIdx.x & 63);
    const double *__restrict__ p = src + ((size_t)wave * rows + (size_t)(lane < rows ? lane : 0)) * (size_t)cols;
    double acc = 0.0;
    for (int t = 0; t < cols; t++)
        acc += lane < rows ? p[t] : 0.0;
    if (acc == 0x1.23456789abcdep+700)
        sink[0] = acc;
}

__global__ __launch_bounds__(256) void k_fill_ceiling(uint4 *__restrict__ dst, size_t n16, uint32_t seed)
{
    const size_t stride = (size_t)gridDim.x * blockDim.x;
    for (size_t i = (size_t)blockIdx.x * blockDim.x + threadIdx.x; i < n16; i += stride) {
        const uint32_t v = seed + (uint32_t)i;
        dst[i] = make_uint4(v, v ^ 0x00010001u, v + 0x00020002u, v ^ 0x7fff7fffu);
    }
}

__global__ __launch_bounds__(256) void k_end_states_to_host(const uint4 *__restrict__ src, uint4 *__restrict__ dst_host, size_t n16,
                                                            const uint32_t *__restrict__ status, uint32_t *__restrict__ status_host)
{
    const size_t stride = (size_t)gridDim.x * blockDim.x;
    for (size_t i = (size_t)blockIdx.x * blockDim.x + threadIdx.x; i < n16; i += stride)
        dst_host[i] = src[i];
    if (blockIdx.x == 0 && threadIdx.x == 0)
        *status_host = *status;
}

typedef unsigned int gather_u32x4 __attribute__((ext_vector_type(4)));
__global__ __launch_bounds__(256) void k_gather_to_host(const gather_u32x4 *__restrict__ src, gather_u32x4 *__restrict__ dst_host, size_t n16)
{
    const size_t per = 256 * 4;
    const size_t nchunk = (n16 + per - 1) / per;
    for (size_t c = blockIdx.x; c < nchunk; c += gridDim.x) {
        const size_t base = c * per + threadIdx.x;
        gather_u32x4 v[4];
#pragma unroll
        for (int u = 0; u < 4; u++)
            if (base + (size_t)u * 256 < n16)
                v[u] = __builtin_nontemporal_load(src + base + (size_t)u * 256);
#pragma unroll
        for (int u = 0; u < 4; u++)
            if (base + (size_t)u * 256 < n16)
                __builtin_nontemporal_store(v[u], dst_host + base + (size_t)u * 256);
    }
}

constexpr int PACK_SC8 = 1, PACK_SC1 = 2;
constexpr int PACK_UNITS = 2048;
constexpr size_t PACK_CHUNK = PACK_UNITS * 8;
typedef unsigned int pack_u32x2 __attribute__((ext_vector_type(2)));

__device__ __forceinline__ uint32_t pack_sc8(int v, int shift, uint32_t &clip)
{
    const int s = v >> shift;
    const int c = min(max(s, -128), 127);
    clip += c != s;
    return (uint32_t)c & 0xffu;
}
__device__ __forceinline__ uint32_t pack_sc8_word(uint32_t a, uint32_t b, int shift, uint32_t &clip)
{
    return pack_sc8((int)(a << 16) >> 16, shift, clip) | pack_sc8((int)a >> 16, shift, clip) << 8 |
           pack_sc8((int)(b << 16) >> 16, shift, clip) << 16 | pack_sc8((int)b >> 16, shift, clip) << 24;
}
__device__ __forceinline__ uint32_t pack_sc1(gather_u32x4 q)
{
    const uint32_t w[4] = {q.x, q.y, q.z, q.w};
    uint32_t r = 0;
#pragma unroll
    for (int k = 0; k < 4; k++)
        r |= (uint32_t)((int)(w[k] << 16) > 0) << (7 - 2 * k) | (uint32_t)((int)w[k] > 0x0000ffff) << (6 - 2 * k);
    return r;
}

template <int FMT>
__global__ __launch_bounds__(256) void k_pack_iq(const int16_t *__restrict__ src, unsigned char *__restrict__ dst, size_t n, int shift,
                                                 unsigned long long *__restrict__ clip)
{
    __shared__ __attribute__((aligned(16))) unsigned char t1[FMT == PACK_SC1 ? PACK_UNITS : 16];
    __shared__ uint32_t wsum[4];
    const int tid = (int)threadIdx.x;
    uint32_t cl = 0;
    const size_t nunits = n / 8;
    if ((((uintptr_t)src & 15) | ((uintptr_t)dst & 7)) == 0) {
        const gather_u32x4 *__restrict__ sv = reinterpret_cast<const gather_u32x4 *>(src);
        const size_t nchunk = (nunits + PACK_UNITS - 1) / PACK_UNITS;
        for (size_t c = blockIdx.x; c < nchunk; c += gridDim.x) {
            const size_t u0 = c * PACK_UNITS + (size_t)tid;
            gather_u32x4 v[8];
#pragma unroll
            for (int u = 0; u < 8; u++)
                if (u0 + (size_t)u * 256 < nunits)
                    v[u] = __builtin_nontemporal_load(sv + u0 + (size_t)u * 256);
            if (FMT == PACK_SC8) {
#pragma unroll
                for (int u = 0; u < 8; u++)
                    if (u0 + (size_t)u * 256 < nunits) {
                        pack_u32x2 o;
                        o.x = pack_sc8_word(v[u].x, v[u].y, shift, cl);
                        o.y = pack_sc8_word(v[u].z, v[u].w, shift, cl);
                        __builtin_nontemporal_store(o, reinterpret_cast<pack_u32x2 *>(dst) + u0 + (size_t)u * 256);
                    }
            } else {
#pragma unroll
                for (int u = 0; u < 8; u++)
                    if (u0 + (size_t)u * 256 < nunits)
                        t1[u * 256 + tid] = (unsigned char)pack_sc1(v[u]);
                __syncthreads();
                const size_t b0 = c * PACK_UNITS + 8 * (size_t)tid;
                if (b0 + 8 <= nunits) {
// ... 86 lines not shown
```

### pluto-gps-sim_amd/csrc/gpsbb_laps.hip.h

```cpp
#ifndef GPSBB_LAPS_HIP_H
#define GPSBB_LAPS_HIP_H

#include "gpsbb_walk.hip.h"
#include "gpsbb_events.hip.h"

namespace gpsbb_impl {

#ifdef GPSBB_LAP_WAVES
#define GPSBB_LAP_OCC __attribute__((amdgpu_waves_per_eu(GPSBB_LAP_WAVES, GPSBB_LAP_WAVES)))
#else
#define GPSBB_LAP_OCC
#endif
constexpr int LAP_WG = 256;
constexpr uint32_t LAPF_ACTIVE = 1u;
constexpr uint32_t LAPF_HEAD = 2u;
constexpr uint32_t LAPF_CONT = 4u;
constexpr uint32_t LAPF_CONST = 8u;
constexpr uint32_t LAPF_BAD = 16u;
constexpr uint32_t ST_LAP_PLAN = 8u;

struct LapBC {
    double phi;
    double s;
    double R1;
// ... 929 lines not shown
            phi -= range;
            dK = 1;
        }
        if (!known && phi < 0.0) {
            phi += range;
            dK = -1;
        }
        (void)dK;
        int eK = 0;
        double ef = 0.0;
        uint32_t nl = 0;
        if (act) {
            const bool to_end = KIND == NCO_CARR && cont_out;
            lap_advance(s, ds, to_end ? p.nsamp : p.nsamp - 1, range, eK, ef);
            double f = (known && start >= range ? 0.0 : phi) + ef + c_own;
            if (f >= range) {
                f -= range;
                eK++;
            }
            if (f < 0.0) {
                f += range;
                eK--;
            }
            int W = s < 0.0 ? -eK : eK;
            W = W < 0 ? 0 : W;
            const int wmax = to_end ? p.nsamp : p.nsamp - 1;
            W = W > wmax ? wmax : W;
            if (L.unit[KIND] == 0 && (head || known))
                W = 0;
            const uint32_t un = L.unit[KIND] > 0 ? (uint32_t)L.unit[KIND] : 1u;
            nl = ((uint32_t)W + un - 1u) / un + (head || known ? 1u : 0u);
        }
        uint32_t incl = nl;
#pragma unroll
        for (int off = 1; off < 64; off <<= 1) {
            const uint32_t v = __shfl_up(incl, off);
            if (lane >= off)
                incl += v;
        }
        if (in) {
            LapBC o;
            o.phi = phi;
            o.s = s;
            o.R1 = R1;
            {
                double r1 = 0.0;
                o.Rphi = act ? lap_R<KIND>(s, phi >= range ? range : phi, r1) : 0.0;
            }
            o.flags = (act ? LAPF_ACTIVE : 0u) | (known ? LAPF_HEAD : 0u) | (cont_out ? LAPF_CONT : 0u);
            o.c0 = KIND == NCO_CODE && act ? c0_of : 0u;
            bcs[b] = o;
            lane0[b] = lanes_before + incl - nl;
            if (!act && slim) {
                p.lap_end[k] = 0.0;
            } else if (!act) {
                gpsbb_chan_state_t &e = p.end[k];
                if (KIND == NCO_CARR) {
                    e.carr_phase = fixed && prn > 0 ? (double)(uint32_t)(p.kph0[k] + (uint32_t)p.nsamp * (uint32_t)p.kstep[k]) : 0.0;
                } else {
                    e.code_phase = 0.0;
                    e.iword = e.ibit = e.icode = e.dataBit = e.codeCA = 0;
                    e._pad = 0;
                }
            }
        }
        lanes_before += (uint32_t)__shfl((int)incl, 63);
        LapScanEl last;
        last.reset = __shfl(acc.reset, 63);
        last.K = __shfl(acc.K, 63);
        last.phi = __shfl(known ? (start >= range ? 0.0 : start) : acc.phi, 63);
        LapScanEl adv;
        adv.reset = 0;
        adv.K = __shfl(aK, 63);
        adv.phi = __shfl(af, 63);
        carry = lap_scan_combine(last, adv, range);
        carry_c = __shfl(corr + c_own, 63);
    }
    if (lane == 0) {
        lane0[p.nblocks] = lanes_before;
        L.nlaps[KIND * GPSBB_MAX_CHAN + i] = lanes_before;
        L.nbad[KIND * GPSBB_MAX_CHAN + i] = 0;
        const uint32_t room = (L.chunk0[KIND][i + 1] - L.chunk0[KIND][i]) * (uint32_t)LAP_WG;
        if (lanes_before > room) {
            atomicOr(p.status, ST_LAP_PLAN);
            L.nlaps[KIND * GPSBB_MAX_CHAN + i] = 0;
        }
    }
}

__global__ __launch_bounds__(256) void k_lap_fixed_tiles(BatchDev p)
{
    const int bi = blockIdx.x;
    const int b = bi / p.nch, i = bi % p.nch;
    if (p.ch[bi].prn <= 0)
        return;
    double *__restrict__ txf = p.tile_x + ((size_t)b * (2 * (size_t)p.nch) + 2 * i + 1) * (size_t)p.ntiles;
    for (int t = threadIdx.x; t < p.ntiles; t += blockDim.x)
        txf[t] = fixed_tile_index(p.kph0[bi], p.kstep[bi], t);
}


template <int KIND>
__device__ __forceinline__ int lap_channel_of(const LapDev &L, int nch, uint32_t c)
{
    int i = 0;
    while (i + 1 < nch && c >= L.chunk0[KIND][i + 1])
        i++;
    return i;
}

constexpr int LAP_WAVES = LAP_WG / 64;
struct LapPassLds {
    double A[LAP_WAVES + 1];
    double m[LAP_WAVES + 1];
    int32_t b[LAP_WAVES + 1], n0[LAP_WAVES + 1];
    uint32_t head[LAP_WAVES + 1];
    double wg[LAP_WAVES];
    uint32_t wo[LAP_WAVES];
    int wc[LAP_WAVES];
};
__device__ __forceinline__ double lap_next(double v, double edge, int lane)
{
    const double d = __shfl_down(v, 1);
    return lane == 63 ? edge : d;
}
__device__ __forceinline__ int32_t lap_next(int32_t v, int32_t edge, int lane)
{
    const int32_t d = __shfl_down(v, 1);
    return lane == 63 ? edge : d;
}

template <int KIND>
__device__ __forceinline__ LapLane<KIND> lap_lane(bool on, double x, int32_t b, int32_t n0, uint32_t jc, bool has_next, int32_t nb, int32_t nn0)
{
    LapLane<KIND> w;
    w.x = x;
    w.s = 0.0;
    w.b = b;
    w.n = n0;
    w.bt = has_next ? nb : INT32_MAX;
    w.nt = has_next ? nn0 : 0;
    w.nmax = 0;
    w.es = 0;
    w.tiemask = 0ull;
    w.jc = jc;
    w.c0 = 0;
    w.navt = 0;
    w.bits = 0;
    w.hz = 0;
    w.bcflags = 0;
    w.outcome = 0;
    w.so = 0;
    w.tt = false;
    w.one_lap = false;
    w.acc = lap_identity();
    w.active = on;
    w.neg = false;
    w.fresh = true;
    return w;
}

template <int KIND>
__device__ __forceinline__ uint32_t lap_jc_of(const BatchDev &p, const LapDev &L, int i, uint32_t r, int32_t b_start)
{
    if (KIND != NCO_CODE)
        return 0u;
    const uint32_t *lane0 = L.lane0 + ((size_t)KIND * p.nch + i) * ((size_t)p.nblocks + 1);
// ... 476 lines not shown
```

### pluto-gps-sim_amd/csrc/gpsbb_plan.h

```cpp
#ifndef GPSBB_PLAN_H
#define GPSBB_PLAN_H

struct BatchPlan {
    int nblocks = 0, nch = 0, nsamp = 0, ntiles = 0;
    double delt = 0.0;
    unsigned flags = 0;
    bool ev = false, ev_dense = false, ev_all_dense = false;
    bool laps = false;
    bool host_seed = false;
    int st_log2 = 0, nstates = 0;
    bool chain_dev = false;
    bool chain_starts = false;
    bool chain_indep = false;
    bool chain_model = false;
    bool chain_fix_seq = false;
    int nseg = 1, seg_tiles = 0;
    int fix_wg = FIXP_WG_BATCH, fix_chunks = 0;
    int nsets = 2;
    uint64_t total_rows = 0;
    int seed_lanes = 0;
    int carr_lanes = 0;
    int chain_lanes = 0;
    uint32_t cont0_mask = 0;
    uint32_t lap_chunk0[2][GPSBB_MAX_CHAN + 1] = {};
};

struct PlanImages {
    std::vector<gpsbb_chan_t> h_ch;
    std::vector<EvConst> h_evc;
    std::vector<uint64_t> row_off;
    std::vector<uint32_t> h_kph0;
    std::vector<int32_t> h_kstep;
    std::vector<ChainDesc> h_cd;
    std::vector<double> h_start0;
    std::vector<int32_t> h_seed_order;
    std::vector<int32_t> h_chain_order;
};

struct StreamLink {
    ChainCarryDev *d_carry = nullptr;
    const int *carry_prn = nullptr;
    double *carry_phase = nullptr;
    hipEvent_t ev_prefix = nullptr, ev_fix = nullptr;
    unsigned stream_turn = 0;
    const int *fixed_prev_prn = nullptr;
    const uint32_t *fixed_prev_phase = nullptr;
};


constexpr size_t HOST_SEED_MAX_CHANNELS = 64;
constexpr int CHAIN_ONLY_BLOCKS = 16384;
constexpr double CHAIN_ONLY_LAPS = 6.0e6;

struct PlanIn {
    const gpsbb_chan_t *ch;
    int nblocks, nch;
    double delt;
    int nsamp;
    unsigned flags;
};

struct PlanOpts {
    int seed_where = 0, synth_kernel = 0, chain_where = 0;
    bool skip_seed = false;
    int max_sets = NSETS;
    bool no_laps = false, device_seed_only = false;
    size_t host_seed_max = HOST_SEED_MAX_CHANNELS;
    long state_log2 = 0, indep_min_tiles = 0, seg_rows = 0, walk_lanes = 0;
    long nsets[2] = {3, 4};
    int chain_only_blocks = CHAIN_ONLY_BLOCKS;
    double chain_only_laps = CHAIN_ONLY_LAPS;
};

static PlanOpts plan_opts(int seed_where, int synth_kernel, bool skip_seed, int chain_where, int max_sets)
{
    PlanOpts o;
    o.seed_where = seed_where;
    o.synth_kernel = synth_kernel;
    o.skip_seed = skip_seed;
    o.chain_where = chain_where;
    o.max_sets = max_sets;
    o.no_laps = GPSBB_KNOB_SET("GPSBB_NO_LAPS");
    o.device_seed_only = GPSBB_KNOB_SET("GPSBB_DEVICE_SEED_ONLY");
    o.host_seed_max = (size_t)GPSBB_KNOB_LONG("GPSBB_HOST_SEED_MAX", HOST_SEED_MAX_CHANNELS);
    o.state_log2 = GPSBB_KNOB_LONG("GPSBB_EV_STATE_LOG2", GPSBB_EV_STATE_LOG2);
    o.indep_min_tiles = GPSBB_KNOB_LONG("GPSBB_INDEP_MIN_TILES", CHAIN_INDEP_MIN_TILES);
    o.seg_rows = GPSBB_KNOB_LONG("GPSBB_SEG_ROWS", CHAIN_SEG_ROWS);
    o.walk_lanes = GPSBB_KNOB_LONG("GPSBB_WALK_LANES", 64);
    o.nsets[0] = GPSBB_KNOB_LONG("GPSBB_NSETS", 3);
    o.nsets[1] = GPSBB_KNOB_LONG("GPSBB_NSETS", 4);
    o.chain_only_blocks = (int)std::min(std::max(GPSBB_KNOB_LONG("GPSBB_CHAIN_ONLY_BLOCKS", CHAIN_ONLY_BLOCKS), 1L), (long)CHAIN_ONLY_BLOCKS);
    o.chain_only_laps = (double)std::min(std::max(GPSBB_KNOB_LONG("GPSBB_CHAIN_ONLY_LAPS", CHAIN_ONLY_LAPS), 1L), (long)CHAIN_ONLY_LAPS);
    return o;
}

static PlanOpts plan_opts(const gpsbb *h, int max_sets)
{
    return plan_opts(h->opt_seed_where, h->opt_synth_kernel, h->opt_skip_seed, h->opt_chain_where, max_sets);
}

static void plan_kernel(BatchPlan &pl, PlanImages &img, const PlanIn &in, const PlanOpts &o)
{
    const gpsbb_chan_t *ch = in.ch;
    const size_t nbc = (size_t)in.nblocks * in.nch;
    const bool fixed = (in.flags & GPSBB_FIXED_CARRIER) != 0;
    pl.ev = o.synth_kernel != 1 && ev_plan(ch, in.nblocks, in.nch, in.delt, img.h_evc, fixed);
    pl.ev_dense = false;
    pl.ev_all_dense = pl.ev;
    if (pl.ev)
        for (size_t k = 0; k < nbc; k++) {
            pl.ev_dense = pl.ev_dense || img.h_evc[k].kc == EV_KC_DENSE;
            pl.ev_all_dense = pl.ev_all_dense && (ch[k].prn <= 0 || img.h_evc[k].kc == EV_KC_DENSE);
        }
    pl.ev_all_dense = pl.ev_all_dense && pl.ev_dense;
    if (fixed && pl.ev_dense && !pl.ev_all_dense) {
        pl.ev = false;
        pl.ev_dense = pl.ev_all_dense = false;
    }
    PUSH_MARK("ev_plan");
}

static int plan_begin(BatchPlan &pl, PlanImages &img, const PlanIn &in, const PlanOpts &o)
{
    if (!in.ch || in.nblocks < 1 || in.nblocks > 65535 || in.nch < 1 || in.nch > GPSBB_MAX_CHAN || in.nsamp < 1 ||
        !(in.delt > 0.0) || !std::isfinite(in.delt) || (in.flags & ~(GPSBB_CHAIN_CARRIER | GPSBB_FIXED_CARRIER)))
        return GPSBB_E_BADARG;
    const size_t nbc = (size_t)in.nblocks * in.nch;
    for (size_t k = 0; k < nbc; k++)
        if (!chan_ok(in.ch[k], in.delt, (in.flags & GPSBB_FIXED_CARRIER) != 0))
// ... 679 lines not shown
```

### pluto-gps-sim_amd/csrc/gpsbb_testhooks.h

```cpp
#ifndef GPSBB_TESTHOOKS_H
#define GPSBB_TESTHOOKS_H
#include <stdint.h>
#ifdef __cplusplus
extern "C" {
#endif

typedef struct gpsbb_test_row {
    int32_t n0;
    uint32_t nav;
    uint64_t xb;
    int64_t inc;
} gpsbb_test_row_t;

double gpsbb_test_carr_jump(double x, double s, long long n);
double gpsbb_test_code_jump(double x, double s, long long n, long long *wraps);
int gpsbb_test_build_rows(int kind, double x0, double s, unsigned nav0, int nsamp, gpsbb_test_row_t *rows,
                          int cap, double *x_end, unsigned *nav_end);
int gpsbb_test_build_rows_f64(int kind, double x0, double s, unsigned nav0, int nsamp, gpsbb_test_row_t *rows,
                              int cap, double *x_end, unsigned *nav_end);
unsigned long long gpsbb_test_row_bound(int kind, double s_abs, int nsamp);
double gpsbb_test_carr_predict(double x0, double s, int n);
double gpsbb_test_fixed_tile_index(unsigned ph0, int step, int t);

#define GPSBB_TEST_PLAN_NQ 38
struct gpsbb_chan;
int gpsbb_test_plan(const struct gpsbb_chan *ch, int nblocks, int nch, double delt, int nsamp, unsigned flags, const int opt[5],
                    int carry, const int *carry_prn, double *carry_phase, const int *fixed_prev_prn,
                    const uint32_t *fixed_prev_phase, unsigned long long out[GPSBB_TEST_PLAN_NQ]);
#define GPSBB_TEST_LAUNCH_NF 29
#define GPSBB_TEST_LAUNCH_KERNELS 16
#define GPSBB_TEST_LAUNCH_NQ (GPSBB_TEST_LAUNCH_NF + 1 + 5 * GPSBB_TEST_LAUNCH_KERNELS)
int gpsbb_test_launch_plan(const struct gpsbb_chan *ch, int nblocks, int nch, double delt, int nsamp, unsigned flags, const int opt[5],
                           int carry, const int *carry_prn, double *carry_phase, const int *fixed_prev_prn,
                           const uint32_t *fixed_prev_phase, int cus, int want_digest, int skip, long long out[GPSBB_TEST_LAUNCH_NQ]);
int gpsbb_test_push_side(const struct gpsbb_chan *ch, int nblocks, int nch, double delt, int nsamp, unsigned flags, const int opt[5],
                         int out[2]);
#define GPSBB_TEST_CHAIN_PLAN_PIECES 64
#define GPSBB_TEST_CHAIN_PLAN_NQ (4 + 4 * GPSBB_TEST_CHAIN_PLAN_PIECES)
int gpsbb_test_chain_plan(const struct gpsbb_chan *ch, int nblocks, int nch, double delt, int nsamp, int seed_where,
                          unsigned long long out[GPSBB_TEST_CHAIN_PLAN_NQ]);

#define GPSBB_TEST_ME_NQ 11
#define GPSBB_TEST_MEC_NQ 4
struct gpsbb_batch;
int gpsbb_test_model_err(struct gpsbb_batch *b, double *maxima, unsigned long long *counts, int *which);
unsigned long long gpsbb_test_despread_exact(struct gpsbb_batch *b);
float gpsbb_test_despread_ms(struct gpsbb_batch *b);
float gpsbb_test_acquire_ms(struct gpsbb *h);
float gpsbb_test_track_ms(struct gpsbb *h);
float gpsbb_test_fir_ms(struct gpsbb *h);
int gpsbb_test_fir_tile(void);
float gpsbb_test_psd_ms(struct gpsbb *h);
int gpsbb_test_psd_run(int log2n);
float gpsbb_test_exc_ms(struct gpsbb *h);
int gpsbb_test_exc_run(int log2n);
int gpsbb_test_exc_host(const gpsbb_exc_t *e, const int16_t *w, long nsamp, const int16_t *hist_in, int16_t *out, int16_t *hist_out,
                        uint64_t *clipped, uint64_t *excised, int64_t *peak);
float gpsbb_test_blank_ms(struct gpsbb *h);
int gpsbb_test_blank_tile(int *run);
void gpsbb_test_blank_nt(int on);
int gpsbb_test_blank_host(const gpsbb_blank_t *b, const int16_t *w, long nsamp, const int16_t *hist_in, int16_t *out, int16_t *hist_out,
                          uint64_t *blanked, uint64_t *triggers);
int gpsbb_test_state_log2(struct gpsbb_batch *b);
int gpsbb_test_state_log2_carr(struct gpsbb_batch *b);
void gpsbb_test_budgets(double out[3]);
void gpsbb_test_nav_sign(unsigned long long state_bits, int minus, int g, int e, int used, long long out[6]);
void gpsbb_test_live(long long out[3]);

#ifdef __cplusplus
}
#endif
#endif
```

### pluto-gps-sim_amd/csrc/gpsbb_walk.hip.h

```cpp
#ifndef GPSBB_WALK_HIP_H
#define GPSBB_WALK_HIP_H

#include "gpsbb_kernels.hip.h"

namespace gpsbb_impl {

#ifndef GPSBB_WALK_WG
#define GPSBB_WALK_WG 64
#endif
constexpr int WALK_ROW_MAX = 4 * TILE - 1;

struct WalkRow {
    int32_t n0;
    uint32_t nav;
    double x;
};
static_assert(sizeof(WalkRow) == 16 && sizeof(WalkRow) <= sizeof(SynRow), "rows of the walk live in the SynRow pool");

__device__ __forceinline__ double walk_row_step(double x, double s)
{
    const uint32_t hi = (uint32_t)__double2hiint(x);
    const double C = __hiloint2double((int)((hi & 0xfff00000u) | 0x80000u), 0);
    return add_rn(add_rn(s, C), -C);
}

template <int KIND>
struct WalkLane {
    double x, s;
    int32_t n;
    uint32_t nav;
    uint32_t bits;
    const uint32_t *dwrd;
    WalkRow *rows;
    uint32_t cap, cnt;
    bool active;
    bool stuck;
    ChainAux *aux;
    int32_t ncross;
    int32_t prev_ex;
    double prev_x1;
    bool prev_wrapped;
    bool prev_tie;
    bool tie_done;
    bool wrap_seen;
    double margin;
    uint32_t hz512;
};

__device__ __forceinline__ uint32_t walk_dbits(const uint32_t *dwrd, uint32_t nav, uint32_t cur)
{
    const uint32_t nav1 = nav_advance(nav);
    const uint32_t nxt = nav_icode(nav1) == 0 ? (nav_bit(dwrd, nav1) < 0 ? 2u : 0u) : (cur ? 2u : 0u);
    return (cur ? 1u : 0u) | nxt;
}

__device__ __forceinline__ int walk_tie_d(uint64_t sb)
{
    const uint64_t Ms = (sb & F64_MANT) | F64_HID;
    return __builtin_ctzll(Ms) + 1;
}
__device__ __forceinline__ uint64_t walk_tiemask(uint64_t sb)
{
    const int d = walk_tie_d(sb);
    return d >= 2 && d <= 50 ? 1ull << d : 0ull;
}

template <int KIND, bool SNEG, bool TRACK, bool STORE = true>
__device__ __forceinline__ void walk_lockstep(WalkLane<KIND> &w, int nsamp, unsigned long long *hz, uint32_t *status)
{
    constexpr int TOPEX = KIND == NCO_CARR ? 1023 : 1023 + 10;
    const double s = w.s;
    const uint64_t sb = f64_bits(s);
    const int es = (int)((sb >> 52) & 0x7ff);
    const bool generic = es < 123;
    const uint64_t tiemask = generic ? 0ull : walk_tiemask(sb);
    const bool any_tie = __ballot(w.active && tiemask != 0ull) != 0ull;
    const bool ttf = TRACK && SNEG && KIND == NCO_CARR && !generic && walk_tie_d(sb) == 1022 - es;
    while (__ballot(w.active)) {
        const double x = w.x;
        const uint32_t hi = (uint32_t)__double2hiint(x);
        const int ex = (int)(hi >> 20);
        const int d = ex - es;
        const bool weird = (unsigned)(ex - 1) >= (unsigned)(TOPEX - 1);
        const bool rare = w.active && (w.stuck || (!weird && (generic || d > 50)));
        bool expl = weird || d < 2;
        const bool first_wrap_row = TRACK && KIND == NCO_CARR && w.active && w.prev_wrapped && !w.wrap_seen;
        if (TRACK && SNEG)
            expl |= ttf && first_wrap_row;
        if (any_tie)
            expl |= ((tiemask >> (d & 63)) & 1ull) != 0ull && (__double2loint(x) & 1);
        const double C = __hiloint2double((int)((hi & 0xfff00000u) | 0x80000u), 0);
        double S = add_rn(add_rn(s, C), -C);
        double room;
        if (!SNEG) {
            double lim = __hiloint2double((int)(hi | 0xfffffu), -1);
            if (KIND == NCO_CODE)
                lim = ex == 1023 + 9 ? 0x1.ff7ffffffffffp+9  : lim;
            room = add_rn(lim, -x);
        } else {
            room = add_rn(x, -__hiloint2double((int)(hi & 0xfff00000u), 1));
        }
        const double Sa = SNEG ? -S : S;
        const double kq = fmin(room * __builtin_amdgcn_rcp(Sa), 4096.0);
        int ki = (int)kq;
        const double rem = __fma_rn(-(double)ki, Sa, room);
        ki += (rem < 0.0 ? -1 : 0) + (rem >= Sa ? 1 : 0);
        const int kleft = nsamp - w.n;
        const int kcap = kleft < WALK_ROW_MAX ? kleft : WALK_ROW_MAX;
        int k = (expl || !(room >= Sa)) ? 0 : (ki < kcap ? ki : kcap);
        double x1 = __fma_rn((double)k, S, x);
        if (TRACK) {
            const double lo = __hiloint2double((int)(hi & 0xfff00000u), 0);
            const double dl = add_rn(SNEG ? x1 : x, -lo), dh = add_rn(add_rn(lo, lo), -(SNEG ? x : x1));
            w.margin = w.active ? fmin(w.margin, (weird || rare) ? 0.0 : fmin(dl, dh)) : w.margin;
            if (KIND == NCO_CARR) {
                const bool cross = w.active && ((!w.wrap_seen && (ex > w.prev_ex || w.prev_wrapped)) || (w.prev_tie && !w.tie_done));
                if (__builtin_expect(__ballot(cross) != 0ull, 0)) {
                    if (cross && w.prev_tie) {
                        atomicAdd(hz + 5, 1ull);
                        w.tie_done = w.wrap_seen;
                    }
                    if (cross) {
                        if (w.ncross >= 0 && w.ncross < CHAIN_MAX_CROSS) {
                            w.aux->cross[w.ncross] = w.n;
                            w.aux->pre[w.ncross] = w.prev_x1;
                            w.aux->post[w.ncross] = x;
                            w.ncross++;
                        } else {
                            w.ncross = -1;
                        }
                        if (w.prev_wrapped && !w.wrap_seen) {
                            w.aux->wrap_row = w.n;
                            w.aux->wrap_x = x;
                        }
                        w.wrap_seen = w.wrap_seen || w.prev_wrapped;
                    }
                }
                w.prev_ex = w.active ? ex : w.prev_ex;
            }
        }
        if (__builtin_expect(__ballot(rare || (w.active && weird)) != 0ull, 0)) {
            if (KIND == NCO_CARR && w.active && ex >= TOPEX && !(hi >> 31))
                w.hz512++;
            if (rare && w.stuck) {
                k = kcap;
                S = 0.0;
                x1 = x;
            } else if (rare) {
                int64_t inc;
                const uint64_t xb = f64_bits(x);
                k = (int)regular_run<KIND>(xb, sb, (int64_t)kcap, inc);
                S = step_of_inc(xb, inc);
                x1 = bits_f64(xb + (uint64_t)((int64_t)k * inc));
            }
        }
        const bool keeps = w.n == 0 || ((uint32_t)(w.n + k) / (uint32_t)TILE) != ((uint32_t)(w.n - 1) / (uint32_t)TILE);
        if (STORE && w.active && keeps) {
            if (w.cnt < w.cap) {
                WalkRow row;
                row.n0 = w.n;
                row.nav = w.bits;
                row.x = x;
                w.rows[w.cnt] = row;
            } else {
                atomicOr(status, ST_ROW_OVERFLOW);
            }
            w.cnt++;
        }
        const int n1 = w.n + k;
        const bool step = w.active && n1 < nsamp;
        double x2 = add_rn(x1, s);
        bool wrapped, tie = false;
        if (KIND == NCO_CARR) {
            wrapped = SNEG ? x2 < 0.0 : x2 >= 1.0;
            const double xw = add_rn(x2, SNEG ? 1.0 : -1.0);
            if (SNEG && TRACK)
                tie = (wrapped && fabs(add_rn(add_rn(xw, -1.0), -x2)) == 0x1p-54) || (ttf && first_wrap_row);
            if (!SNEG && TRACK)
                tie = wrapped && fabs(add_rn(add_rn(x2, -x1), -s)) == 0x1p-53;
#ifdef GPSBB_EXP_NOTIE
            tie = false;
#endif
            x2 = wrapped ? xw : x2;
        } else {
            wrapped = x2 >= 1023.0;
            x2 = wrapped ? add_rn(x2, -1023.0) : x2;
            if (__ballot(step && wrapped)) {
                if (step && wrapped) {
                    w.nav = nav_advance(w.nav);
                    uint32_t cur = w.bits & 1u;
                    if (nav_icode(w.nav) == 0) {
                        if (nav_iword(w.nav) >= GPSBB_N_DWRD)
                            atomicAdd(hz + 1, 1ull);
                        cur = nav_bit(w.dwrd, w.nav) < 0 ? 1u : 0u;
                    }
                    w.bits = walk_dbits(w.dwrd, w.nav, cur);
                }
            }
        }
        if (__builtin_expect(__ballot(rare || (w.active && weird)) != 0ull, 0))
            w.stuck = (rare || weird) && step && !wrapped && f64_bits(x2) == f64_bits(x1);
        w.x = step ? x2 : (w.active ? x1 : w.x);
        w.n = step ? n1 + 1 : (w.active ? n1 : w.n);
        if (KIND == NCO_CARR && TRACK) {
            w.prev_wrapped = w.active ? (step && wrapped) : w.prev_wrapped;
            w.prev_tie = w.active ? (step && tie) : w.prev_tie;
            const bool last_cross = step && !(w.n < nsamp) &&
                                    ((!w.wrap_seen && (wrapped || (int)((uint32_t)__double2hiint(x2) >> 20) > ex)) || (tie && !w.tie_done));
            if (__builtin_expect(__ballot(last_cross) != 0ull, 0)) {
                if (last_cross) {
                    if (w.ncross >= 0 && w.ncross < CHAIN_MAX_CROSS) {
                        w.aux->cross[w.ncross] = nsamp;
                        w.aux->pre[w.ncross] = x1;
                        w.aux->post[w.ncross] = x2;
                        w.ncross++;
                    } else {
                        w.ncross = -1;
                    }
                }
            }
            w.prev_x1 = w.active ? x1 : w.prev_x1;
        }
        w.active = step && w.n < nsamp;
    }
}

template <int KIND, bool TRACK, bool STORE = true>
__device__ __forceinline__ void walk_both_signs(WalkLane<KIND> &w, int nsamp, unsigned long long *hz, uint32_t *status)
{
    const bool on = w.active;
    const bool neg = w.s < 0.0;
    if (__ballot(on && !neg)) {
        w.active = on && !neg;
        walk_lockstep<KIND, false, TRACK, STORE>(w, nsamp, hz, status);
    }
    if (KIND == NCO_CARR && __ballot(on && neg)) {
        w.active = on && neg;
        walk_lockstep<KIND, true, TRACK, STORE>(w, nsamp, hz, status);
    }
}

template <int KIND, bool STORE = true>
__device__ __forceinline__ WalkLane<KIND> walk_lane(const BatchDev &p, int chain, double x0, double s, bool on)
{
    WalkLane<KIND> w;
    w.x = x0;
    w.s = s;
    w.n = 0;
    w.nav = 0;
    w.bits = 0;
    w.dwrd = nullptr;
    w.rows = nullptr;
    w.cap = 0;
    if (STORE) {
        const uint64_t o0 = p.row_off[chain], o1 = p.row_off[chain + 1];
        w.rows = reinterpret_cast<WalkRow *>(p.rows) + o0;
        w.cap = (uint32_t)(o1 - o0);
    }
    w.cnt = 0;
    w.active = on;
    w.stuck = false;
    w.aux = nullptr;
    w.ncross = 0;
    w.prev_ex = 0x7fff;
    w.prev_x1 = 0.0;
    w.prev_wrapped = false;
    w.prev_tie = false;
    w.tie_done = false;
    w.wrap_seen = false;
    w.margin = 1.0;
    w.hz512 = 0;
    return w;
}

template <int PASS>
__global__ __launch_bounds__(GPSBB_WALK_WG) void k_walk(BatchDev p)
{
    __builtin_amdgcn_s_setprio(GPSBB_SEED_PRIO);
    const int gid = blockIdx.x * blockDim.x + threadIdx.x;
    const int nbc = p.nblocks * p.nch;
    int c = -1;
    if (gid < p.seed_lanes) {
        if (p.seed_order) {
            c = p.seed_order[gid];
        } else {
            const int nbp = (p.nvb + 63) & ~63;
            const int i = gid / nbp, b = gid - i * nbp;
            c = (i < p.nch && b < p.nvb) ? nbc + b * p.nch + i : -1;
        }
    }
    const bool is_code = c >= 0 && c < nbc, is_carr = c >= nbc;
    if (PASS != 1 && PASS != 3 && __ballot(is_code)) {
        const int k = is_code ? c : 0;
        const gpsbb_chan_t &ch = p.ch[k];
        const bool on = is_code && ch.prn > 0;
        WalkLane<NCO_CODE> w = walk_lane<NCO_CODE>(p, k, ch.code_phase, mul_rn(ch.f_code, p.delt), on);
        w.nav = nav_pack(ch.icode, ch.ibit, ch.iword);
        w.dwrd = ch.dwrd;
        w.bits = on ? walk_dbits(ch.dwrd, w.nav, nav_bit(ch.dwrd, w.nav) < 0 ? 1u : 0u) : 0u;
        walk_both_signs<NCO_CODE, false>(w, p.nsamp, p.hazards, p.status);
        if (is_code) {
            gpsbb_chan_state_t &e = p.end[k];
            p.row_cnt[k] = on ? (int32_t)(w.cnt < w.cap ? w.cnt : w.cap) : 0;
            if (on) {
                e.code_phase = w.x;
                e.iword = nav_iword(w.nav);
                e.ibit = nav_ibit(w.nav);
                e.icode = nav_icode(w.nav);
                e.dataBit = nav_bit(ch.dwrd, w.nav);
                const int ci = (int)w.x;
                e.codeCA = (int)((p.ca_bits[ch.prn * 32 + (ci >> 5)] >> (ci & 31)) & 1u) * 2 - 1;
            } else {
                e.code_phase = 0.0;
                e.iword = e.ibit = e.icode = e.dataBit = e.codeCA = 0;
            }
            e._pad = 0;
        }
    }
    if (__ballot(is_carr)) {
        const int k = is_carr ? c - nbc : 0;
        const int prn = PASS >= 1 ? p.cd[k].prn : p.ch[k].prn;
        const double f_carr = PASS >= 1 ? p.cd[k].f_carr : p.ch[k].f_carr;
        const bool fx = PASS == 0 && p.kph0 != nullptr;
        const bool on = is_carr && prn > 0 && !fx;
        const double x0 = PASS == 1 ? p.start0[k] : (PASS >= 2 ? (p.model_start ? p.start0[k] : p.aux[k].start1) : p.ch[k].carr_phase);
        const int vb = k / p.nch, sgi = PASS >= 1 ? vb % p.nseg : 0;
        const int ns = PASS >= 1 ? seg_nsamp(p, sgi) : p.nsamp;
        WalkLane<NCO_CARR> w = walk_lane<NCO_CARR, PASS == 0 || PASS == 2>(p, nbc + k, x0, mul_rn(f_carr, p.delt) , on);
        w.aux = PASS >= 2 ? &p.aux[k] : nullptr;
        if (PASS >= 2)
            walk_both_signs<NCO_CARR, true, PASS == 2>(w, ns, p.hazards, p.status);
        else
            walk_both_signs<NCO_CARR, false, PASS != 1>(w, ns, p.hazards, p.status);
        if (is_carr) {
            if (PASS == 1) {
                p.aux[k].endA = on ? w.x : 0.0;
            } else {
                if (PASS != 3) {
                    p.row_cnt[nbc + k] = on ? (int32_t)(w.cnt < w.cap ? w.cnt : w.cap) : 0;
                    if (PASS == 0)
                        p.end[k].carr_phase = fx ? (prn > 0 ? (double)(uint32_t)(p.kph0[k] + (uint32_t)p.nsamp * (uint32_t)p.kstep[k]) : 0.0)
                                                 : (on ? w.x : 0.0);
                }
                if (PASS >= 2) {
                    ChainAux &a = p.aux[k];
                    a.margin = w.margin;
                    a.ncross = on ? w.ncross : 0;
                    if (!w.wrap_seen)
                        a.wrap_row = -1;
                    a.prefix_cnt = 0;
                    a.endB = on ? w.x : 0.0;
                    p.aux[k].hz512 = on ? w.hz512 : 0u;
                } else if (on && w.hz512) {
                    atomicAdd(p.hazards, (unsigned long long)w.hz512);
                }
            }
        }
    }
}

__device__ __forceinline__ bool chain_continues(const BatchDev &p, int b, int i)
{
    const ChainDesc &d = p.cd[(size_t)b * p.nch + i];
    if (b == 0)
        return p.carry && d.prn > 0 && ((p.cont0_mask >> i) & 1u);
    return d.prn > 0 && !d.start && d.prn == p.cd[(size_t)(b - 1) * p.nch + i].prn;
}

constexpr int PREFIX_WG = 256;
__global__ __launch_bounds__(PREFIX_WG) void k_chain_prefix(BatchDev p)
{
    __shared__ double wv[PREFIX_WG / 64];
    __shared__ int wf[PREFIX_WG / 64];
    __shared__ double carry_s;
    __builtin_amdgcn_s_setprio(3);
    const int i = blockIdx.x, t = threadIdx.x, lane = t & 63, wave = t >> 6;
    if (i >= p.nch)
        return;
    double carry = 0.0;
    for (int b0 = 0; b0 < p.nvb; b0 += PREFIX_WG) {
        const int b = b0 + t;
        const bool in = b < p.nvb;
        const size_t k = (size_t)(in ? b : 0) * p.nch + i;
        const bool cont = in && chain_continues(p, b, i);
        const double start0 = in ? p.start0[k] : 0.0;
        double c = 0.0;
        if (cont) {
            c = (b == 0 ? p.carry->approx_end[i] : p.aux[k - p.nch].endA) - start0;
            c = c > 0.5 ? c - 1.0 : (c < -0.5 ? c + 1.0 : c);
        }
        double v = c;
        bool f = !cont;
#pragma unroll
        for (int o = 1; o < 64; o <<= 1) {
            const double vu = __shfl_up(v, o);
            const int fu = __shfl_up((int)f, o);
            if (lane >= o) {
                v = f ? v : v + vu;
                f = f || fu;
            }
        }
        if (lane == 63) {
            wv[wave] = v;
            wf[wave] = f ? 1 : 0;
        }
        __syncthreads();
        for (int w = wave - 1; w >= 0 && !f; w--) {
            v += wv[w];
            f = wf[w] != 0;
        }
        const double e = f ? v : v + carry;
        if (in) {
            ChainAux &a = p.aux[k];
            double st = cont ? start0 + e : p.cd[k].carr_phase;
            st = st >= 1.0 ? st - 1.0 : (st < 0.0 ? st + 1.0 : st);
            a.start1 = st;
// ... 148 lines not shown
            double pre_j = 0.0, post_j = 0.0;
            if (j >= FIX_PREFETCH_CROSS) {
                pre_j = a.pre[j];
                post_j = a.post[j];
            } else {
#pragma unroll
                for (int q = 0; q < FIX_PREFETCH_CROSS; q++) {
                    pre_j = j == q ? in.pre[q] : pre_j;
                    post_j = j == q ? in.post[q] : post_j;
                }
            }
            double xt = pre_j + d;
            carr_step(xt, s);
            d = xt - post_j;
            ok = fabs(d) < margin - 0x1p-51;
            if (COMMIT)
                a.seg[j + 1] = d;
        }
    } else if (base && !ok && in.wrap_row >= 0) {
        const int nstar = in.wrap_row;
        const FixWalkOut lap = (COMMIT && !p.chain_starts)
                                   ? fix_walk<true>(x, s, nstar, reinterpret_cast<WalkRow *>(p.prefix_rows) + k * CHAIN_PREFIX_CAP, CHAIN_PREFIX_CAP)
                                   : fix_walk<false>(x, s, nstar, nullptr, p.chain_starts ? 0x7fffffffu : (uint32_t)CHAIN_PREFIX_CAP);
        const bool overflow = lap.overflow;
        const uint32_t lap_rows = lap.cnt, lap_hz = lap.hz512;
        d = lap.x - in.wrap_x;
        ok = !overflow && lap_hz == 0 && fabs(d) < margin - 0x1p-51 &&
             !(tie_top && fmod(fabs(d) * (fall ? 0x1p+53 : 0x1p+52), 2.0) != 0.0);
        if (ok) {
            const double d_wrap = d;
            int m = 1;
            for (int j = 0; ok && j < ncross; j++) {
                const int cj = a.cross[j];
                if (cj <= nstar)
                    continue;
                double xt = a.pre[j] + d;
                carr_step(xt, s);
                d = xt - a.post[j];
                ok = fabs(d) < margin - 0x1p-51;
                if (COMMIT) {
                    a.cross[m] = cj;
                    a.seg[m + 1] = d;
                }
                m++;
            }
            if (ok && COMMIT) {
                a.prefix_cnt = (int32_t)lap_rows;
                a.prefix_end = nstar;
                a.ncross = m;
                a.cross[0] = nstar;
                a.seg[0] = 0.0;
                a.seg[1] = d_wrap;
            }
        }
    }
    if (on && ok && d0 != 0.0)
        end = end + d;
#ifdef GPSBB_CHAIN_DEBUG
    if (COMMIT && on && p.nch == 1) {
        printf("fix k %d x %.17g start1 %.17g d0 %.3e margin %.3e ncross %d wrap_row %d tie_top %d tie_asc %d ok %d endB %.17g end %.17g s %.17g\n",
               (int)k, x, in.start1, d0, margin, ncross, in.wrap_row, (int)tie_top, (int)tie_asc, (int)ok, in.endB, end, s);
        for (int j = 0; j < ncross && j < CHAIN_MAX_CROSS; j++)
            printf("    cross %d sample %d pre %.17g post %.17g seg %.3e\n", j, a.cross[j], a.pre[j], a.post[j], a.seg[j + 1]);
    }
#endif
    if (on && !ok) {
        if (!run_slow) {
            out.kind = FIX_SLOW;
            out.end = end;
            out.hz512 = 0;
            return out;
        }
        out.walked = true;
        if (p.chain_starts) {
            end = fix_walk<false>(x, s, nsamp_seg, nullptr, 0x7fffffffu).x;
        } else {
            const uint32_t cap = (uint32_t)(p.row_off[nbc + k + 1] - p.row_off[nbc + k]);
            WalkRow *rows = reinterpret_cast<WalkRow *>(p.rows) + p.row_off[nbc + k];
            const FixWalkOut w = COMMIT ? fix_walk<true>(x, s, nsamp_seg, rows, cap) : fix_walk<false>(x, s, nsamp_seg, nullptr, cap);
            end = w.x;
            hz512 = w.hz512;
            if (COMMIT) {
                if (w.overflow)
                    atomicOr(p.status, ST_ROW_OVERFLOW);
                p.row_cnt[nbc + k] = (int32_t)(w.cnt < cap ? w.cnt : cap);
                a.ncross = 0;
                a.seg[0] = 0.0;
                a.prefix_cnt = 0;
            }
        }
    }
    out.end = end;
    out.hz512 = hz512;
    return out;
}

__device__ __forceinline__ void fix_publish(const BatchDev &p, size_t k, bool on, bool cont, double x, const FixOut &r,
                                            unsigned long long &n_hz)
{
    const size_t vb = k / (size_t)p.nch, i = k % (size_t)p.nch;
    const size_t kb = (vb / (size_t)p.nseg) * (size_t)p.nch + i;
    const int sgi = (int)(vb % (size_t)p.nseg);
    if (p.chain_starts) {
        if (on && cont) {
            p.cd[k].carr_phase = x;
            if (p.ch && sgi == 0)
                const_cast<gpsbb_chan_t *>(p.ch)[kb].carr_phase = x;
        }
    } else {
        if (sgi == p.nseg - 1)
            p.end[kb].carr_phase = on ? r.end : 0.0;
        if (on)
            n_hz += r.hz512;
    }
}

__global__ __launch_bounds__(64) void k_chain_fix(BatchDev p)
{
    __builtin_amdgcn_s_setprio(3);
    const int i = threadIdx.x;
    const bool lane_on = i < p.nch;
    const int il = lane_on ? i : 0;
    double prev_end = p.carry ? p.carry->exact_end[il] : 0.0;
    unsigned long long n_fallback = 0, n_hz = 0;
    FixIn nxt = fix_load(p, 0, il);
    FixIn nxt2 = fix_load(p, p.nvb > 1 ? 1 : 0, il);
    for (int b = 0; b < p.nvb; b++) {
        const FixIn in = nxt;
        nxt = nxt2;
        nxt2 = fix_load(p, b + 2 < p.nvb ? b + 2 : p.nvb - 1, il);
        const size_t k = (size_t)b * p.nch + il;
        const bool on = lane_on && in.prn > 0;
        const bool cont = on && (b > 0 ? in.prn == in.prn_prev : (p.carry && ((p.cont0_mask >> il) & 1u)));
        const double x = cont ? prev_end : in.carr_phase;
        const FixOut r = fix_block<true>(p, in, k, on, x, true);
        n_fallback += r.walked ? 1u : 0u;
        if (lane_on)
            fix_publish(p, k, on, cont, x, r, n_hz);
        prev_end = r.end;
    }
    if (p.carry && lane_on)
        p.carry->exact_end[i] = prev_end;
    if (n_hz)
        atomicAdd(p.hazards, n_hz);
    if (n_fallback)
        atomicAdd(p.hazards + 4, n_fallback);
}

constexpr int FIXP_WG_BATCH = 128, FIXP_WG_ALONE = 256;

struct FixMap {
    int isconst;
    double v[4];
};
__device__ __forceinline__ FixMap fix_compose(const FixMap &A, const FixMap &B)
{
    FixMap R;
    if (A.isconst)
        return A;
    if (B.isconst) {
        const double o = B.v[0];
        const int cls = (int)fmax(fmin(o, 0x1p+30), -0x1p+30) & 3;
        double add = A.v[0];
        add = cls == 1 ? A.v[1] : add;
        add = cls == 2 ? A.v[2] : add;
        add = cls == 3 ? A.v[3] : add;
        R.isconst = 1;
// ... 56 lines not shown
    const double endB_prev = (mine && b > 0) ? p.aux[k - p.nch].endB : 0.0;
    FixMap my;
    my.isconst = 0;
    my.v[0] = my.v[1] = my.v[2] = my.v[3] = 0.0;
    bool have = false;
    double x_last = 0.0, my_end = 0.0;
    FixOut r_last;
    r_last.end = 0.0;
    r_last.kind = FIX_OK;
    r_last.hz512 = 0;
    r_last.walked = false;
    if (mine && !on) {
        my.isconst = 1;
    } else if (on) {
        const bool known = !cont || b == 0;
        const double xk = (cont && b == 0) ? p.carry->exact_end[i] : in.carr_phase;
        bool regular = true;
        double kk[4] = {0.0, 0.0, 0.0, 0.0};
#pragma unroll 1
        for (int j = 0; j < (known ? 1 : 4) && regular; j++) {
            const double xj = known ? xk : endB_prev + (double)j * 0x1p-53;
            const FixOut r = fix_block<false>(p, in, k, on, xj, false);
            const double o = (r.end - in.endB) * 0x1p+53;
            if (known) {
                have = true;
                x_last = xj;
                r_last = r;
                kk[0] = r.kind == FIX_OK ? o : 0.0;
            } else {
                regular = r.kind == FIX_OK && fabs(o) < 0x1p+30 && o == __builtin_rint(o);
                const double kj = o - (double)j;
                kk[0] = j == 0 ? kj : kk[0];
                kk[1] = j == 1 ? kj : kk[1];
                kk[2] = j == 2 ? kj : kk[2];
                kk[3] = j == 3 ? kj : kk[3];
            }
        }
        if (known || !regular) {
            my.isconst = 1;
            my.v[0] = known ? kk[0] : 0.0;
        } else {
#pragma unroll
            for (int j = 0; j < 4; j++)
                my.v[j] = kk[j];
        }
    }
    FixMap acc = my;
#pragma unroll
    for (int off = 1; off < 64; off <<= 1) {
        const FixMap prev = fix_map_shfl_up(acc, off);
        if (lane >= off)
            acc = fix_compose(acc, prev);
    }
    if (lane == 63) {
        L.wc[wave] = acc.isconst;
#pragma unroll
        for (int j = 0; j < 4; j++)
            L.wv[wave][j] = acc.v[j];
    }
    if (t == 0) {
        L.first_bad = FIXP_WG;
        L.head_end = endB_prev;
    }
    __syncthreads();
    for (int w = wave - 1; w >= 0 && !acc.isconst; w--) {
        FixMap pw;
        pw.isconst = L.wc[w];
#pragma unroll
        for (int j = 0; j < 4; j++)
            pw.v[j] = L.wv[w][j];
        acc = fix_compose(acc, pw);
    }
    const double endB_before = L.head_end;
    __syncthreads();
    if (t == 0) {
        double cs = p.carry ? p.carry->exact_end[i] : 0.0;
        if (chunk > 0) {
            const size_t at = (size_t)i * p.fix_chunks + (chunk - 1);
            __builtin_amdgcn_s_setprio(0);
            unsigned long long spins = 0;
            while (__hip_atomic_load(&p.fix_flag[at], __ATOMIC_ACQUIRE, __HIP_MEMORY_SCOPE_AGENT) != p.fix_epoch) {
                __builtin_amdgcn_s_sleep(32);
                if (++spins > (1ull << 22)) {
                    atomicOr(p.status, ST_CHAIN_STALL);
                    break;
                }
            }
            __builtin_amdgcn_s_setprio(3);
            cs = bits_f64(__hip_atomic_load(&p.fix_end[at], __ATOMIC_RELAXED, __HIP_MEMORY_SCOPE_AGENT));
        }
        L.head_end = cs;
    }
    __syncthreads();
    const double chunk_start = L.head_end;
    __syncthreads();
    if (chunk > 0) {
        FixMap inc;
        inc.isconst = 1;
        inc.v[0] = (chunk_start - endB_before) * 0x1p+53;
        inc.v[1] = inc.v[2] = inc.v[3] = 0.0;
        acc = fix_compose(acc, inc);
    }
    int lo = -1;
    double lo_start = chunk_start;
    bool committed = false, final = false, pre = true;
    double prev_end = 0.0;
    for (;;) {
        const bool head = t == lo && mine && !final;
        if (head) {
            const double x = cont ? lo_start : in.carr_phase;
            if (!have || f64_bits(x) != f64_bits(x_last)) {
                r_last = fix_block<false>(p, in, k, on, x, false);
                x_last = x;
                have = true;
            }
        }
        const bool commit_now = mine && !committed && (final || (head && r_last.kind == FIX_SLOW));
        if (commit_now) {
            const double x = cont ? (final ? prev_end : lo_start) : in.carr_phase;
            const FixOut r = fix_block<true>(p, in, k, on, x, true);
            committed = true;
            n_fallback += r.walked ? 1u : 0u;
            fix_publish(p, k, on, cont, x, r, n_hz);
            x_last = x;
            r_last = r;
            have = true;
        }
        if (final)
            break;
        if (!pre) {
            if (head) {
                my.isconst = 1;
                my.v[0] = (r_last.end - in.endB) * 0x1p+53;
            }
            acc = my;
            if (t < lo) {
                acc.isconst = 0;
                acc.v[0] = acc.v[1] = acc.v[2] = acc.v[3] = 0.0;
            }
#pragma unroll
            for (int off = 1; off < 64; off <<= 1) {
                const FixMap prev = fix_map_shfl_up(acc, off);
                if (lane >= off)
                    acc = fix_compose(acc, prev);
            }
            if (lane == 63) {
                L.wc[wave] = acc.isconst;
#pragma unroll
                for (int j = 0; j < 4; j++)
                    L.wv[wave][j] = acc.v[j];
            }
            if (t == 0)
                L.first_bad = FIXP_WG;
            __syncthreads();
            for (int w = wave - 1; w >= 0 && !acc.isconst; w--) {
                FixMap pw;
                pw.isconst = L.wc[w];
#pragma unroll
                for (int j = 0; j < 4; j++)
                    pw.v[j] = L.wv[w][j];
                acc = fix_compose(acc, pw);
            }
        }
        pre = false;
        if (mine && t >= lo)
            my_end = t == lo ? r_last.end : in.endB + acc.v[0] * 0x1p-53;
        if (lane == 63)
// ... 140 lines not shown
```

Before: 656.8 billion.

## Skip copy stage for device-resident batches and mirror status flags to pinned host

For batches with no host IQ, digest or level output (lean slots), the pop path now waits on the synth-done event instead of a separate copy event. End states are written to host by a kernel on the prepass stream. Device error flags are also mirrored into a pinned host word through system-scope atomics, so no status copy is needed. Timed runs record synth events through hipExtLaunchKernelGGL instead of separate event records. This removes per-batch copy-stream work and event hops, at the cost of extra system-scope atomics on error paths and more complex synchronization.

```diff
diff --git a/pluto-gps-sim_amd/csrc/gpsbb.hip b/pluto-gps-sim_amd/csrc/gpsbb.hip
--- a/pluto-gps-sim_amd/csrc/gpsbb.hip
+++ b/pluto-gps-sim_amd/csrc/gpsbb.hip
@@ -1,4 +1,5 @@
 #include <hip/hip_runtime.h>
+#include <hip/hip_ext.h>
 
 #include <algorithm>
 #include <atomic>
@@ -553,6 +554,7 @@
     DevBuf<int32_t> d_tabs;
     DevBuf<uint32_t> d_ca;
     DevBuf<uint32_t> d_status;
+    PinnedBuf<uint32_t> h_status;
     DevBuf<unsigned long long> d_hz;
     DevBuf<unsigned long long> d_clip;
     DevBuf<int2> d_noise_tab;
@@ -961,7 +963,7 @@
     h->host_regs.clear();
     chain_only_free(h);
     (void)drain_streams(h);
-    release_all(h->d_tabs, h->d_ca, h->d_status, h->d_hz, h->d_clip, h->d_noise_tab, h->d_nclip);
+    release_all(h->d_tabs, h->d_ca, h->d_status, h->h_status, h->d_hz, h->d_clip, h->d_noise_tab, h->d_nclip);
     release_all(h->d_pack, h->d_level, h->d_digest, h->d_acq_chips, h->d_acq_rows, h->d_acq_grid, h->d_trk, h->d_fir, h->d_psd_tab, h->d_psd, h->d_exc, h->d_blank);
     release_all(h->acq_tm, h->trk_tm, h->fir_tm, h->psd_tm, h->exc_tm, h->blank_tm);
     delete h->pool;
@@ -994,6 +996,12 @@
 #endif
     const hipError_t e = hipMemsetAsync(ptr, 0, bytes, h->s_seed);
     return e != hipSuccess ? e : hipStreamSynchronize(h->s_seed);
+}
+
+static hipError_t status_clear(gpsbb *h)
+{
+    *h->h_status.p = 0;
+    return zero_now(h, h->d_status.p, 4);
 }
 
 struct SynthKernel {
@@ -1050,6 +1058,8 @@
     if ((e = (hipError_t)h->d_tabs.reserve(sizeof tabs / sizeof tabs[0])) != hipSuccess) return fail(e);
     if ((e = (hipError_t)h->d_ca.reserve(ca.size())) != hipSuccess) return fail(e);
     if ((e = (hipError_t)h->d_status.reserve(1)) != hipSuccess) return fail(e);
+    if ((e = (hipError_t)h->h_status.reserve(1)) != hipSuccess) return fail(e);
+    *h->h_status.p = 0;
     if ((e = (hipError_t)h->d_hz.reserve(8)) != hipSuccess) return fail(e);
     if ((e = (hipError_t)h->d_clip.reserve(1)) != hipSuccess) return fail(e);
     if ((e = hipMemcpy(h->d_tabs.p, tabs, sizeof tabs, hipMemcpyHostToDevice)) != hipSuccess) return fail(e);
@@ -1579,6 +1589,7 @@
     p.kstep = (pl.flags & GPSBB_FIXED_CARRIER) ? b->d_kstep.p : nullptr;
     p.end = ts.end.p;
     p.status = b->h->d_status.p;
+    p.status_host = b->h->h_status.p;
     p.hazards = b->h->d_hz.p;
     p.digest = b->want_digest ? b->d_dig.p : nullptr;
     p.seed_order = b->d_seed_order.p;
@@ -1768,10 +1779,15 @@
     return GPSBB_OK;
 }
 
-static int synth_launch(gpsbb_batch *b, const BatchDev &p, const LaunchPlan &lp, hipStream_t sc, int16_t *d_iq)
+static bool ring_packets() { return GPSBB_KNOB_LONG("GPSBB_RING_PACKETS", 0) != 0; }
+
+static int synth_launch(gpsbb_batch *b, const BatchDev &p, const LaunchPlan &lp, hipStream_t sc, int16_t *d_iq, const Event *ev_synth)
 {
     const SynthKernel &k = synth_kernel(lp.variant, lp.digest_fused, lp.granule);
-    hipLaunchKernelGGL(k.fn, dim3(lp.grid_x, lp.grid_y), dim3(lp.wg), k.lds, sc, p, d_iq);
+    if (ev_synth)
+        hipExtLaunchKernelGGL(k.fn, dim3(lp.grid_x, lp.grid_y), dim3(lp.wg), (uint32_t)k.lds, sc, ev_synth[0].e, ev_synth[1].e, 0u, p, d_iq);
+    else
+        hipLaunchKernelGGL(k.fn, dim3(lp.grid_x, lp.grid_y), dim3(lp.wg), k.lds, sc, p, d_iq);
     if (lp.digest_gx)
         hipLaunchKernelGGL(k_block_digest, dim3(lp.digest_gx, lp.digest_gy), dim3(256), 0, sc, (const uint32_t *)d_iq, b->plan.nsamp, b->d_dig.p);
     HIPCHK(b->h, hipGetLastError());
@@ -1808,6 +1824,16 @@
     if (rc != GPSBB_OK)
         return rc;
     HIPCHK(h, hipGetLastError());
+    if (b->link.h_end) {
+        const size_t bytes = (size_t)pl.nblocks * pl.nch * sizeof(gpsbb_chan_state_t);
+        hipLaunchKernelGGL(k_end_states_to_host, dim3(64), dim3(256), 0, ss, (const uint4 *)ts.end.p, (uint4 *)b->link.h_end,
+                           (bytes + 15) / 16, (const uint32_t *)nullptr, (uint32_t *)nullptr);
+        HIPCHK(h, hipGetLastError());
+    }
+#ifdef GPSBB_EXPERIMENTS
+    if (b->link.raise)
+        hipLaunchKernelGGL(k_status_raise, dim3(1), dim3(64), 0, ss, h->d_status.p, h->h_status.p);
+#endif
     if (timed)
         HIPCHK(h, hipEventRecord(ev[1], ss));
     h->last_prepass = lp.info_prepass;
@@ -1828,14 +1854,15 @@
         HIPCHK(h, hipStreamWaitEvent(sc, ev[1], 0));
     if (!lp.ctr_reset)
         HIPCHK(h, hipMemsetAsync(p.tile_ctr, 0, ((size_t)pl.nblocks + 1) * sizeof(int32_t), sc));
-    if (timed)
+    const bool on_dispatch = timed && !b->want_digest && !ring_packets();
+    if (timed && !on_dispatch)
         HIPCHK(h, hipEventRecord(ev[2], sc));
     if (b->want_digest)
         HIPCHK(h, hipMemsetAsync(b->d_dig.p, 0, (size_t)pl.nblocks * sizeof(unsigned long long), sc));
-    rc = synth_launch(b, p, lp, sc, d_iq);
+    rc = synth_launch(b, p, lp, sc, d_iq, on_dispatch ? ev + 2 : nullptr);
     if (rc != GPSBB_OK)
         return rc;
-    if (timed)
+    if (timed && !on_dispatch)
         HIPCHK(h, hipEventRecord(ev[3], sc));
     ts.synth_done_ref = ev[3];
     b->last_done = ev[3];
@@ -1874,7 +1901,7 @@
     uint32_t st = 0;
     HIPCHK(h, hipMemcpy(&st, h->d_status.p, 4, hipMemcpyDeviceToHost));
     if (st) {
-        HIPCHK(h, zero_now(h, h->d_status.p, 4));
+        HIPCHK(h, status_clear(h));
         return GPSBB_E_INTERNAL;
     }
     return GPSBB_OK;
@@ -3319,7 +3346,7 @@
     if (end_state)
         memcpy(end_state, h->h_fill.p, (size_t)nch * sizeof(gpsbb_chan_state_t));
     if (*st) {
-        HIPCHK(h, zero_now(h, h->d_status.p, 4));
+        HIPCHK(h, status_clear(h));
         return GPSBB_E_INTERNAL;
     }
     return GPSBB_OK;
@@ -3551,6 +3578,8 @@
         PinnedBuf<LevelOut> h_lvl;
         bool has_lvl = false;
         Event computed, copied;
+        hipEvent_t popped_at = nullptr;
+        bool lean = false;
         void release()
         {
             if (batch)
@@ -3819,6 +3848,11 @@
 {
     gpsbb *h = s->h;
     gpsbb_batch *b = sl.batch;
+    if (sl.lean) {
+        sl.popped_at = b->last_done;
+        return GPSBB_OK;
+    }
+    sl.popped_at = sl.copied;
     hipStream_t cs = b->last_cs;
     if (sl.h_iq.p) {
         if (!h->s_copy)
@@ -3910,6 +3944,12 @@
         b->link.fixed_prev_prn = s->chain.fx_prn;
         b->link.fixed_prev_phase = s->chain.fx_phase;
     }
+    sl.lean = !sl.h_iq.p && !want_digest && !want_level && !ring_packets();
+    if (sl.lean)
+        b->link.h_end = sl.h_end.p;
+#ifdef GPSBB_EXPERIMENTS
+    b->link.raise = GPSBB_KNOB_LONG("GPSBB_RAISE_AT_PUSH", -1) == (long)s->head;
+#endif
     PUSH_MARK("plan");
     hipStream_t us = nullptr;
     HIPCHK(h, batch_prepass_stream(b, b->link.d_carry != nullptr, &us));
@@ -3980,7 +4020,7 @@
     gpsbb *h = s->h;
     HIPCHK(h, hipSetDevice(h->device));
     auto &sl = s->slots[s->tail % s->depth];
-    HIPCHK(h, hipEventSynchronize(sl.copied));
+    HIPCHK(h, hipEventSynchronize(sl.popped_at));
     *iq = sl.h_iq.p ? reinterpret_cast<const int16_t *>(sl.h_iq.p) : sl.batch->d_iq.p;
     if (end_state)
         memcpy(end_state, sl.h_end.p, (size_t)s->bps * s->nch * sizeof(gpsbb_chan_state_t));
@@ -3990,9 +4030,12 @@
         memcpy(levels, sl.h_lvl.p, (size_t)s->bps * sizeof(gpsbb_level_t));
     s->tail++;
     uint32_t st = 0;
-    memcpy(&st, sl.h_end.p + (((size_t)s->bps * s->nch * sizeof(gpsbb_chan_state_t) + 15) & ~(size_t)15), 4);
+    if (sl.lean)
+        st = __atomic_load_n(h->h_status.p, __ATOMIC_ACQUIRE);
+    else
+        memcpy(&st, sl.h_end.p + (((size_t)s->bps * s->nch * sizeof(gpsbb_chan_state_t) + 15) & ~(size_t)15), 4);
     if (st) {
-        HIPCHK(h, zero_now(h, h->d_status.p, 4));
+        HIPCHK(h, status_clear(h));
         return GPSBB_E_INTERNAL;
     }
     return GPSBB_OK;
@@ -4630,6 +4673,39 @@
 extern "C" float gpsbb_test_track_ms(gpsbb *h) { return h ? h->trk_tm.ms() : -1.0f; }
 extern "C" float gpsbb_test_fir_ms(gpsbb *h) { return h ? h->fir_tm.ms() : -1.0f; }
 
+extern "C" int gpsbb_test_ext_event_probe(gpsbb *h, long long out[6], float ms[3])
+{
+    if (!h || !out || !ms)
+        return GPSBB_E_BADARG;
+    HIPCHK(h, hipSetDevice(h->device));
+    DevBuf<uint32_t> d;
+    PinnedBuf<uint32_t> hw;
+    Event e0, e_begin, e_end;
+    const AtExit done{[&] { (void)drain_streams(h); release_all(d, hw, e0, e_begin, e_end); }};
+    HIPCHK(h, (hipError_t)d.reserve(4));
+    HIPCHK(h, (hipError_t)hw.reserve(2));
+    HIPCHK(h, zero_now(h, d.p, 16));
+    hw.p[0] = hw.p[1] = 0;
+    for (Event *e : {&e0, &e_begin, &e_end})
+        HIPCHK(h, e->make(hipEventDefault));
+    const auto t0 = std::chrono::steady_clock::now();
+    HIPCHK(h, hipEventRecord(e0, h->s_seed));
+    hipExtLaunchKernelGGL(k_probe_step, dim3(1), dim3(64), 0u, h->s_compute, e_begin.e, e_end.e, 0u, (const uint32_t *)nullptr, d.p, hw.p, 100000u);
+    HIPCHK(h, hipGetLastError());
+    out[0] = (long long)hipStreamWaitEvent(h->s_seed, e_end, 0);
+    hipLaunchKernelGGL(k_probe_step, dim3(1), dim3(64), 0, h->s_seed, (const uint32_t *)d.p, d.p + 2, hw.p + 1, 1u);
+    HIPCHK(h, hipGetLastError());
+    out[1] = (long long)hipEventSynchronize(e_end);
+    out[2] = (long long)__atomic_load_n(hw.p, __ATOMIC_ACQUIRE);
+    ms[2] = std::chrono::duration<float, std::milli>(std::chrono::steady_clock::now() - t0).count();
+    HIPCHK(h, hipStreamSynchronize(h->s_seed));
+    out[3] = (long long)__atomic_load_n(hw.p + 1, __ATOMIC_ACQUIRE);
+    ms[0] = ms[1] = -1.0f;
+    out[4] = (long long)hipEventElapsedTime(&ms[0], e_begin, e_end);
+    out[5] = (long long)hipEventElapsedTime(&ms[1], e0, e_end);
+    return GPSBB_OK;
+}
+
 extern "C" int gpsbb_test_fir_tile(void) { return FIR_TILE; }
 extern "C" float gpsbb_test_psd_ms(gpsbb *h) { return h ? h->psd_tm.ms() : -1.0f; }
 extern "C" int gpsbb_test_psd_run(int log2n) { return log2n < PSD_MIN_LOG2N || log2n > PSD_MAX_LOG2N ? -1 : psd_min_run(log2n); }
diff --git a/pluto-gps-sim_amd/csrc/gpsbb_events.hip.h b/pluto-gps-sim_amd/csrc/gpsbb_events.hip.h
--- a/pluto-gps-sim_amd/csrc/gpsbb_events.hip.h
+++ b/pluto-gps-sim_amd/csrc/gpsbb_events.hip.h
@@ -569,7 +569,7 @@
 #endif
     if (lds_addr_of(smem_raw) != 0u) {
         if (tid == 0)
-            atomicOr(p.status, ST_LDS_LAYOUT);
+            status_raise(p.status, p.status_host, ST_LDS_LAYOUT);
         return;
     }
 #ifdef GPSBB_WG_TRACE
diff --git a/pluto-gps-sim_amd/csrc/gpsbb_kernels.hip.h b/pluto-gps-sim_amd/csrc/gpsbb_kernels.hip.h
--- a/pluto-gps-sim_amd/csrc/gpsbb_kernels.hip.h
+++ b/pluto-gps-sim_amd/csrc/gpsbb_kernels.hip.h
@@ -34,6 +34,14 @@
 constexpr uint32_t ST_ROW_OVERFLOW = 1u;
 constexpr uint32_t ST_LDS_LAYOUT = 4u;
 constexpr uint32_t ST_CHAIN_STALL = 2u;
+constexpr uint32_t ST_TEST_RAISE = 16u;
+
+__device__ __forceinline__ void status_raise(uint32_t *status, uint32_t *status_host, uint32_t bits)
+{
+    atomicOr(status, bits);
+    if (status_host)
+        __hip_atomic_fetch_or(status_host, bits, __ATOMIC_RELAXED, __HIP_MEMORY_SCOPE_SYSTEM);
+}
 
 struct SynRow {
     int32_t n0;
@@ -161,6 +169,7 @@
     int seed_lanes;
     const int32_t *seed_order;
     uint32_t *status;
+    uint32_t *status_host;
     unsigned long long *digest;
     unsigned long long *hazards;
     int ev;
@@ -438,7 +447,7 @@
         x = build_rows_f64<NCO_CODE>(c.code_phase, s, nav, p.nsamp, sink);
         sink.finish();
         if (sink.overflow)
-            atomicOr(p.status, ST_ROW_OVERFLOW);
+            status_raise(p.status, p.status_host, ST_ROW_OVERFLOW);
         d.rows = sink.rows;
         d.cnt = (int)sink.cnt;
     }
@@ -478,7 +487,7 @@
         x = build_rows_f64<NCO_CARR>(x0, s, nav, p.nsamp, sink);
         sink.finish();
         if (sink.overflow)
-            atomicOr(p.status, ST_ROW_OVERFLOW);
+            status_raise(p.status, p.status_host, ST_ROW_OVERFLOW);
         d.rows = sink.rows;
         d.cnt = (int)sink.cnt;
     }
@@ -1097,9 +1106,31 @@
     const size_t stride = (size_t)gridDim.x * blockDim.x;
     for (size_t i = (size_t)blockIdx.x * blockDim.x + threadIdx.x; i < n16; i += stride)
         dst_host[i] = src[i];
-    if (blockIdx.x == 0 && threadIdx.x == 0)
+    if (status && blockIdx.x == 0 && threadIdx.x == 0)
         *status_host = *status;
 }
+
+#ifdef GPSBB_EXPERIMENTS
+__global__ __launch_bounds__(64) void k_status_raise(uint32_t *status, uint32_t *status_host)
+{
+    if (threadIdx.x == 0)
+        status_raise(status, status_host, ST_TEST_RAISE);
+}
+
+__global__ __launch_bounds__(64) void k_probe_step(const uint32_t *seen, uint32_t *out_dev, uint32_t *out_host, uint32_t turns)
+{
+    if (threadIdx.x != 0)
+        return;
+    uint32_t x = turns;
+    for (uint32_t i = 0; i < turns; i++)
+        x = x * 1664525u + 1013904223u;
+    const uint32_t v = (seen ? __hip_atomic_load(seen, __ATOMIC_RELAXED, __HIP_MEMORY_SCOPE_AGENT) : 0u) + 1u;
+    out_dev[1] = x;
+    out_dev[0] = v;
+    if (out_host)
+        *out_host = v;
+}
+#endif
 
 typedef unsigned int gather_u32x4 __attribute__((ext_vector_type(4)));
 __global__ __launch_bounds__(256) void k_gather_to_host(const gather_u32x4 *__restrict__ src, gather_u32x4 *__restrict__ dst_host, size_t n16)
diff --git a/pluto-gps-sim_amd/csrc/gpsbb_laps.hip.h b/pluto-gps-sim_amd/csrc/gpsbb_laps.hip.h
--- a/pluto-gps-sim_amd/csrc/gpsbb_laps.hip.h
+++ b/pluto-gps-sim_amd/csrc/gpsbb_laps.hip.h
@@ -1035,7 +1035,7 @@
         L.nbad[KIND * GPSBB_MAX_CHAN + i] = 0;
         const uint32_t room = (L.chunk0[KIND][i + 1] - L.chunk0[KIND][i]) * (uint32_t)LAP_WG;
         if (lanes_before > room) {
-            atomicOr(p.status, ST_LAP_PLAN);
+            status_raise(p.status, p.status_host, ST_LAP_PLAN);
             L.nlaps[KIND * GPSBB_MAX_CHAN + i] = 0;
         }
     }
diff --git a/pluto-gps-sim_amd/csrc/gpsbb_plan.h b/pluto-gps-sim_amd/csrc/gpsbb_plan.h
--- a/pluto-gps-sim_amd/csrc/gpsbb_plan.h
+++ b/pluto-gps-sim_amd/csrc/gpsbb_plan.h
@@ -45,6 +45,8 @@
     unsigned stream_turn = 0;
     const int *fixed_prev_prn = nullptr;
     const uint32_t *fixed_prev_phase = nullptr;
+    void *h_end = nullptr;
+    bool raise = false;
 };
 
 
diff --git a/pluto-gps-sim_amd/csrc/gpsbb_testhooks.h b/pluto-gps-sim_amd/csrc/gpsbb_testhooks.h
--- a/pluto-gps-sim_amd/csrc/gpsbb_testhooks.h
+++ b/pluto-gps-sim_amd/csrc/gpsbb_testhooks.h
@@ -48,6 +48,8 @@
 float gpsbb_test_despread_ms(struct gpsbb_batch *b);
 float gpsbb_test_acquire_ms(struct gpsbb *h);
 float gpsbb_test_track_ms(struct gpsbb *h);
+struct gpsbb;
+int gpsbb_test_ext_event_probe(struct gpsbb *h, long long out[6], float ms[3]);
 float gpsbb_test_fir_ms(struct gpsbb *h);
 int gpsbb_test_fir_tile(void);
 float gpsbb_test_psd_ms(struct gpsbb *h);
diff --git a/pluto-gps-sim_amd/csrc/gpsbb_walk.hip.h b/pluto-gps-sim_amd/csrc/gpsbb_walk.hip.h
--- a/pluto-gps-sim_amd/csrc/gpsbb_walk.hip.h
+++ b/pluto-gps-sim_amd/csrc/gpsbb_walk.hip.h
@@ -66,7 +66,7 @@
 }
 
 template <int KIND, bool SNEG, bool TRACK, bool STORE = true>
-__device__ __forceinline__ void walk_lockstep(WalkLane<KIND> &w, int nsamp, unsigned long long *hz, uint32_t *status)
+__device__ __forceinline__ void walk_lockstep(WalkLane<KIND> &w, int nsamp, unsigned long long *hz, uint32_t *status, uint32_t *status_host)
 {
     constexpr int TOPEX = KIND == NCO_CARR ? 1023 : 1023 + 10;
     const double s = w.s;
@@ -163,7 +163,7 @@
                 row.x = x;
                 w.rows[w.cnt] = row;
             } else {
-                atomicOr(status, ST_ROW_OVERFLOW);
+                status_raise(status, status_host, ST_ROW_OVERFLOW);
             }
             w.cnt++;
         }
@@ -226,17 +226,17 @@
 }
 
 template <int KIND, bool TRACK, bool STORE = true>
-__device__ __forceinline__ void walk_both_signs(WalkLane<KIND> &w, int nsamp, unsigned long long *hz, uint32_t *status)
+__device__ __forceinline__ void walk_both_signs(WalkLane<KIND> &w, int nsamp, unsigned long long *hz, uint32_t *status, uint32_t *status_host)
 {
     const bool on = w.active;
     const bool neg = w.s < 0.0;
     if (__ballot(on && !neg)) {
         w.active = on && !neg;
-        walk_lockstep<KIND, false, TRACK, STORE>(w, nsamp, hz, status);
+        walk_lockstep<KIND, false, TRACK, STORE>(w, nsamp, hz, status, status_host);
     }
     if (KIND == NCO_CARR && __ballot(on && neg)) {
         w.active = on && neg;
-        walk_lockstep<KIND, true, TRACK, STORE>(w, nsamp, hz, status);
+        walk_lockstep<KIND, true, TRACK, STORE>(w, nsamp, hz, status, status_host);
     }
 }
 
@@ -298,7 +298,7 @@
         w.nav = nav_pack(ch.icode, ch.ibit, ch.iword);
         w.dwrd = ch.dwrd;
         w.bits = on ? walk_dbits(ch.dwrd, w.nav, nav_bit(ch.dwrd, w.nav) < 0 ? 1u : 0u) : 0u;
-        walk_both_signs<NCO_CODE, false>(w, p.nsamp, p.hazards, p.status);
+        walk_both_signs<NCO_CODE, false>(w, p.nsamp, p.hazards, p.status, p.status_host);
         if (is_code) {
             gpsbb_chan_state_t &e = p.end[k];
             p.row_cnt[k] = on ? (int32_t)(w.cnt < w.cap ? w.cnt : w.cap) : 0;
@@ -329,9 +329,9 @@
         WalkLane<NCO_CARR> w = walk_lane<NCO_CARR, PASS == 0 || PASS == 2>(p, nbc + k, x0, mul_rn(f_carr, p.delt) , on);
         w.aux = PASS >= 2 ? &p.aux[k] : nullptr;
         if (PASS >= 2)
-            walk_both_signs<NCO_CARR, true, PASS == 2>(w, ns, p.hazards, p.status);
+            walk_both_signs<NCO_CARR, true, PASS == 2>(w, ns, p.hazards, p.status, p.status_host);
         else
-            walk_both_signs<NCO_CARR, false, PASS != 1>(w, ns, p.hazards, p.status);
+            walk_both_signs<NCO_CARR, false, PASS != 1>(w, ns, p.hazards, p.status, p.status_host);
         if (is_carr) {
             if (PASS == 1) {
                 p.aux[k].endA = on ? w.x : 0.0;
@@ -646,7 +646,7 @@
             hz512 = w.hz512;
             if (COMMIT) {
                 if (w.overflow)
-                    atomicOr(p.status, ST_ROW_OVERFLOW);
+                    status_raise(p.status, p.status_host, ST_ROW_OVERFLOW);
                 p.row_cnt[nbc + k] = (int32_t)(w.cnt < cap ? w.cnt : cap);
                 a.ncross = 0;
                 a.seg[0] = 0.0;
@@ -869,7 +869,7 @@
             while (__hip_atomic_load(&p.fix_flag[at], __ATOMIC_ACQUIRE, __HIP_MEMORY_SCOPE_AGENT) != p.fix_epoch) {
                 __builtin_amdgcn_s_sleep(32);
                 if (++spins > (1ull << 22)) {
-                    atomicOr(p.status, ST_CHAIN_STALL);
+                    status_raise(p.status, p.status_host, ST_CHAIN_STALL);
                     break;
                 }
             }
```

After: 656.7 billion. About the same (-0.0%).
